# nantiferov/karpenter-sigs

Measured on AMD Instinct MI355X. Metric: pods/sec in Scheduler.Solve @50k pods x 400 types, higher is better.
Workload: dtype int64; 1 GPU; C2: 50000 resource-only pods x 400 fake.InstanceTypes, 1 NodeClaimTemplate, no limits, empty topology (BenchmarkScheduling shape); pods=50000, instance_types=400, parallelism=replicas1, new_nodeclaims=122

## Files before the change

### include/karpenter_amd.h

```cpp
#ifndef KARPENTER_AMD_H_
#define KARPENTER_AMD_H_

#include <stddef.h>
#include <stdint.h>

#ifdef __cplusplus
extern "C" {
#endif

#define KS_OK 0
#define KS_ERR_PARSE -1
#define KS_ERR_UNSUPPORTED -2
#define KS_ERR_CAPACITY -3
#define KS_ERR_HIP -4
#define KS_ERR_INTERNAL -5
#define KS_ERR_ARG -6

typedef struct ks_problem ks_problem;
typedef struct ks_results ks_results;

typedef struct ks_solve_opts {
  int device;
  int simulation_mode;
  int replicas;
  int timing_only;
  int lds_budget;
  int reserved[3];
} ks_solve_opts;

int ks_problem_create(const char* snapshot_json, size_t len, ks_problem** out);
void ks_problem_free(ks_problem* p);

int ks_problem_save(const ks_problem* p, void** buf, size_t* len);
int ks_problem_create_binary(const void* buf, size_t len, ks_problem** out);
int ks_snapshot_check(const char* snapshot_json, size_t len, size_t* bytes);
int ks_problem_encode_binary(const char* snapshot_json, size_t len, void** buf, size_t* blen);
int ks_problem_check_binary(const void* buf, size_t len);

int ks_problem_inspect(const char* snapshot_json, size_t len, char** dims_json);

int ks_problem_feasibility_rows(ks_problem* p, int which, char** meta_json, uint32_t** words, size_t* n_words);

int ks_problem_queue_inputs(const char* snapshot_json, size_t len, char** out_json);
int ks_problem_queue_readback(ks_problem* p, int32_t** order, int32_t** run_len, size_t* n, int* device_sorted);
int ks_claim_sort_probe(int device, int mode, int pos, int n, int R, int32_t* keys, int32_t* order,
                        const int32_t* claim_tpl, const int64_t* claim_head, int32_t* ptpl, int64_t* phead, int* how);
int ks_rec_headers_run(const int32_t* records, const int32_t* pass_ns, int n_passes, int TW, const int32_t* tpl_beg,
                       int ntpl, int32_t* headers, uint64_t* status, char** verdicts_json, char** meta_json);

int ks_solve(ks_problem* p, const ks_solve_opts* opts, ks_results** out);
void ks_results_free(ks_results* r);

int ks_results_json(const ks_results* r, char** json_out);

int ks_results_num_new_nodeclaims(const ks_results* r);
int ks_results_nodeclaim(const ks_results* r, int i, int* template_index, const int32_t** pods, int* n_pods,
                         const int32_t** instance_types, int* n_instance_types);
int ks_results_num_existing_nodes(const ks_results* r);
int ks_results_existing_node(const ks_results* r, int i, int* state_node_index, const int32_t** pods, int* n_pods);
int ks_results_num_pod_errors(const ks_results* r);
int ks_results_pod_error(const ks_results* r, int i, int* pod_index, const char** message);

typedef struct ks_requirement {
  const char* key;
  const char* op;
  int n_values;
  const char* const* values;
  int has_gt, has_lt;
  int64_t gt, lt;
} ks_requirement;
int ks_results_nodeclaim_requests(const ks_results* r, int i, int* n, const char* const** names,
                                  const char* const** quantities);
int ks_results_nodeclaim_requirements(const ks_results* r, int i, int* n, const ks_requirement** reqs);

double ks_results_kernel_ms(const ks_results* r);
double ks_results_solve_kernel_ms(const ks_results* r);
double ks_results_feasibility_ms(const ks_results* r);
double ks_results_feasibility_bytes(const ks_results* r);
double ks_results_node_feasibility_ms(const ks_results* r);
double ks_results_node_feasibility_bytes(const ks_results* r);
double ks_results_algorithmic_bytes(const ks_results* r);

typedef struct ks_cons ks_cons;
int ks_cons_create(const char* snapshot_json, size_t len, ks_cons** out);
int ks_cons_save(const ks_cons* c, void** buf, size_t* len);
int ks_cons_create_binary(const void* buf, size_t len, ks_cons** out);
int ks_cons_inspect(const char* snapshot_json, size_t len, char** out_json);
int ks_cons_update(ks_cons* c, const char* update_json, size_t len);
int ks_cons_inspect_update(const char* snapshot_json, size_t len, const char* update_json, size_t ulen,
                           char** out_json);
void ks_cons_free(ks_cons* c);
int ks_cons_num_candidates(const ks_cons* c);
int ks_cons_num_sims(const ks_cons* c);
int ks_cons_record_bytes(const ks_cons* c);
int ks_cons_records_per_rank(const ks_cons* c, int world);
int ks_cons_run(ks_cons* c, int rank, int world, const ks_solve_opts* opts, void* records, int records_on_device,
                double* kernel_ms);
#define KS_CONS_ALL_SIMS 1
#define KS_CONS_CANDIDATES 2
#define KS_CONS_NO_SIMS 4
int ks_cons_requirement_words(const ks_cons* c);
int ks_cons_needed_sims(ks_cons* c, const void* records, int world, int flags, int32_t* out, int cap);
int ks_cons_claim_requirements(ks_cons* c, int sim, uint32_t* out);
int ks_cons_decide(ks_cons* c, const void* records, int world, int flags, const uint32_t* rs_table,
                   char** json_out);
typedef struct ks_cons_clock {
  double multi_timeout_s;
  double single_timeout_s;
  double sim_seconds;
} ks_cons_clock;
int ks_cons_decide_clock(ks_cons* c, const void* records, int world, int flags, const uint32_t* rs_table,
                         const ks_cons_clock* clock, char** json_out);
int ks_cons_validate(ks_cons* c, const char* command_json, size_t len, const ks_solve_opts* opts, char** json_out);
#define KS_DISRUPT_EXPIRATION 1
#define KS_DISRUPT_DRIFT 2
int ks_cons_disrupt(ks_cons* c, int method, const ks_solve_opts* opts, int flags, char** json_out);
int ks_cons_inspect_disrupt(const char* snapshot_json, size_t len, const char* update_json, size_t ulen, int method,
                            char** out_json);
int ks_cons_encode_binary(const char* snapshot_json, size_t len, void** buf, size_t* buf_len);
int ks_cons_inspect_disrupt_binary(const void* buf, size_t len, int method, char** out_json, void** resaved,
                                   size_t* resaved_len);
int ks_cons_sim_counters(ks_cons* c, int sim, int64_t* out24);
int ks_cons_sim_counters_n(ks_cons* c, int sim, int64_t* out, int n);
int ks_cons_queue_readback(ks_cons* c, char** meta_json, int32_t** words, size_t* n_words);
int ks_cons_last_reruns(const ks_cons* c);
int ks_cons_last_routes(const ks_cons* c, char** json_out);
double ks_cons_records_alg_bytes(const ks_cons* c, const void* records, int world);

int ks_cluster_state(const char* cluster_json, size_t len, char** state_nodes_json);

void ks_free(void* p);
const char* ks_last_error(void);
int ks_device_count(void);
const char* ks_build_info(void);

#ifdef __cplusplus
}
#endif
#endif
```

### karpenter-sigs_amd/csrc/ks_capi.cpp

```cpp
#include <hip/hip_runtime_api.h>

#include <algorithm>
#include <chrono>
#include <cstring>
#include <memory>
#include <mutex>
#include <string>
#include <vector>

#include "../../include/karpenter_amd.h"
#include "ks_archive.h"
#include "ks_host.h"
#include "ks_runtime.h"
#include "ks_sort_probe.h"

using namespace ks;

static thread_local std::string g_err;
namespace ks {
void set_last_error(const std::string& m) { g_err = m; }

static thread_local std::vector<Route>* g_routes = nullptr;
void route_note(const Route& r) {
  if (g_routes) g_routes->push_back(r);
// ... 950 lines not shown
  return KS_OK;
  API_CATCH
}

extern "C++" {
namespace {
constexpr char kProblemMagic[8] = {'K', 'S', 'P', 'R', 'O', 'B', '0', '5'};
}

void snapshot_header(ArOut& a, const char magic[8]) {
  a.raw(magic, 8);
  uint32_t v[4] = {1u, (uint32_t)sizeof(KsDims), (uint32_t)sizeof(KeyMeta), (uint32_t)sizeof(Host)};
  a.raw(v, sizeof(v));
}
void snapshot_check_header(ArIn& a, const char magic[8]) {
  char m[8];
  uint32_t v[4];
  a.raw(m, 8);
  a.raw(v, sizeof(v));
  if (memcmp(m, magic, 6) == 0 && memcmp(m, magic, 8) != 0)
    throw KsError(KS_ERR_PARSE, "binary snapshot format version " + std::string(m + 6, 2) + ", this build reads version " +
                                    std::string(magic + 6, 2));
  if (memcmp(m, magic, 8) != 0) throw KsError(KS_ERR_PARSE, "not a binary snapshot of this kind");
  if (v[0] != 1u || v[1] != sizeof(KsDims) || v[2] != sizeof(KeyMeta) || v[3] != sizeof(Host))
    throw KsError(KS_ERR_PARSE, "binary snapshot from another build of the library");
}
char* snapshot_bytes(const std::string& s) {
  char* b = (char*)malloc(std::max<size_t>(s.size(), 1));
  if (!b) throw KsError(KS_ERR_CAPACITY, "out of host memory");
  memcpy(b, s.data(), s.size());
  return b;
}
}

int ks_problem_save(const ks_problem* p, void** buf, size_t* len) {
  API_TRY
  if (!p || !buf || !len) throw KsError(KS_ERR_ARG, "null argument");
  ArOut a;
  snapshot_header(a, kProblemMagic);
  host_save(a, const_cast<Host&>(p->host));
  *buf = snapshot_bytes(a.buf);
  *len = a.buf.size();
  return KS_OK;
  API_CATCH
}

int ks_problem_create_binary(const void* buf, size_t len, ks_problem** out) {
  API_TRY
  if (!buf || !out) throw KsError(KS_ERR_ARG, "null argument");
  std::unique_ptr<ks_problem> pb(new ks_problem());
  try {
    ArIn a{(const char*)buf, (const char*)buf + len};
    snapshot_check_header(a, kProblemMagic);
    host_load(a, pb->host);
    if (a.p != a.end) throw KsError(KS_ERR_PARSE, "binary snapshot has trailing bytes");
  } catch (const ArchiveError& e) {
    throw KsError(KS_ERR_PARSE, e.what());
  }
  problem_device_init(pb.get());
  *out = pb.release();
  return KS_OK;
  API_CATCH
}

int ks_snapshot_check(const char* json, size_t len, size_t* bytes) {
  API_TRY
  if (!json) throw KsError(KS_ERR_ARG, "null argument");
  PhaseTimer pt("ks_snapshot_check");
  ksjson::Value root = ksjson::Parser(json, len ? len : strlen(json)).parse();
  Host h;
  h.build(root);
  pt.mark("parse + encode");
  ArOut a;
  host_save(a, h);
  pt.mark("save");
  Host g;
  try {
    ArIn in{a.buf.data(), a.buf.data() + a.buf.size()};
    host_load(in, g);
    pt.mark("load");
    if (in.p != in.end) throw KsError(KS_ERR_INTERNAL, "snapshot reload left bytes");
  } catch (const ArchiveError& e) {
    throw KsError(KS_ERR_INTERNAL, e.what());
  }
  ArOut b;
  host_save(b, g);
  if (bytes) *bytes = a.buf.size();
  if (a.buf != b.buf) throw KsError(KS_ERR_INTERNAL, "snapshot save -> load -> save is not the identity");
  return KS_OK;
  API_CATCH
}

int ks_problem_encode_binary(const char* json, size_t len, void** buf, size_t* blen) {
  API_TRY
  if (!json || !buf || !blen) throw KsError(KS_ERR_ARG, "null argument");
  ksjson::Value root = ksjson::Parser(json, len ? len : strlen(json)).parse();
  Host h;
  h.build(root);
  ArOut a;
  snapshot_header(a, kProblemMagic);
  host_save(a, h);
  *buf = snapshot_bytes(a.buf);
  *blen = a.buf.size();
  return KS_OK;
  API_CATCH
}

int ks_problem_check_binary(const void* buf, size_t len) {
  API_TRY
  if (!buf) throw KsError(KS_ERR_ARG, "null argument");
  Host h;
  try {
    ArIn a{(const char*)buf, (const char*)buf + len};
    snapshot_check_header(a, kProblemMagic);
    host_load(a, h);
    if (a.p != a.end) throw KsError(KS_ERR_PARSE, "binary snapshot has trailing bytes");
  } catch (const ArchiveError& e) {
    throw KsError(KS_ERR_PARSE, e.what());
  }
  return KS_OK;
  API_CATCH
}

int ks_problem_inspect(const char* json, size_t len, char** out) {
  API_TRY
  if (!json || !out) throw KsError(KS_ERR_ARG, "null argument");
  ksjson::Value root = ksjson::Parser(json, len ? len : strlen(json)).parse();
  Host h;
  h.build(root);
  const KsDims& d = h.dims;
  std::string o = "{";
  auto kv = [&](const char* k, long long v) { o += std::string(o.size() > 1 ? "," : "") + "\"" + k + "\":" + std::to_string(v); };
  kv("R", d.R); kv("keys", d.NK); kv("W", d.W); kv("NB", d.NB); kv("RSW", d.RSW); kv("T", d.T); kv("templates", d.NTPL);
  kv("pools", d.NPOOL); kv("nodes", d.N); kv("pods", d.P); kv("states", d.S); kv("uids", d.NU); kv("TW", d.TW);
  kv("Kcap", d.Kcap); kv("taints", (long long)h.taints.size()); kv("G", d.G); kv("G1", d.G1);
  kv("hostQueue", h.hostQueue.empty() ? 0 : 1); kv("hostPorts", (long long)h.hostPortUniverse.size());
  long long nlate = 0;
  for (uint64_t x : h.tab.tg_late) nlate += __builtin_popcountll(x);
  kv("lateGroups", nlate); kv("groupWords", d.GMW); kv("unlabelledNodes", d.tgUnlab);
  kv("lean", d.lean); kv("negReq", d.negReq);
  long long nfail = 0, nshared = 0, nverr = 0;
  for (char x : h.injectFailed) nfail += x ? 1 : 0;
  for (int32_t f : h.tab.pod_flags) {
    nshared += (f & PF_VSHARED) ? 1 : 0;
    nverr += (f & PF_VOLERR) ? 1 : 0;
  }
  kv("volAny", d.volAny); kv("volDrivers", d.VD); kv("volPvcs", d.NVU); kv("volLogCap", d.vLogCap);
  kv("volSharedPods", nshared); kv("volErrorPods", nverr); kv("injectFailed", nfail);
  kv("volStaticMounts", (long long)(h.tab.pod_vsbeg.empty() ? 0 : h.tab.pod_vsbeg.back()));
  std::vector<int32_t> frontBeg, frontPos;
  pareto_fronts(d, h.tab.tpl_it_beg, h.tab.tpl_its, h.tab.it_alloc, frontBeg, frontPos);
  o += ",\"runFuse\":" + std::to_string(run_fuse_build()) + ",\"sortLeaf\":" + std::to_string(sort_leaf_build()) +
       ",\"closedShift\":" + std::to_string(closed_shift_build()) + ",\"tplMasks\":" + std::to_string(tpl_masks_build()) +
       ",\"logRuns\":" + std::to_string(log_runs_build()) + ",\"paretoFronts\":[";
  for (int t = 0; t < d.NTPL; t++) {
    o += t ? ",[" : "[";
    for (int i = frontBeg[(size_t)t]; i < frontBeg[(size_t)t + 1]; i++)
      o += (i > frontBeg[(size_t)t] ? "," : "") + std::to_string(frontPos[(size_t)i]);
    o += "]";
  }
  o += "]";
  o += ",\"plans\":{";
  const size_t budgets[] = {160 * 1024 - 256, 6000, 9000, 14000, 24000, 40000};
  long long fnr = 0;
  for (int32_t f : h.tab.st_flags) fnr += (f & SF_HAS_KEYS) ? 1 : 0;
  KsDims pd = d;
  pd.fnOn = node_rows_on(d, (size_t)fnr);
  auto plan_json = [&](size_t budget, int wide) {
    Plan pl = make_plan(pd, budget, false, wide, (int)frontPos.size());
    return "{\"KO\":" + std::to_string(pl.KO) +
           ",\"KL\":" + std::to_string(pl.KL) + ",\"talloc\":" + std::to_string(pl.talloc) +
           ",\"tsort\":" + std::to_string(pl.tsort) + ",\"tmask\":" + std::to_string(pl.tmask) +
           ",\"tmaskBytes\":" + std::to_string(pl.tmask ? tpl_mask_bytes(d.NTPL, d.TW) : 0) + ",\"lds\":" + std::to_string(pl.lds) + "}";
  };
  for (size_t i = 0; i < sizeof(budgets) / sizeof(budgets[0]); i++)
    o += (i ? ",\"" : "\"") + std::to_string(budgets[i]) + "\":" + plan_json(budgets[i], 0);
  o += "},\"widePlans\":{";
  for (size_t i = 0; i < sizeof(budgets) / sizeof(budgets[0]); i++)
    o += (i ? ",\"" : "\"") + std::to_string(budgets[i]) + "\":[" + plan_json(budgets[i], 1) + "," + plan_json(budgets[i], 2) + "]";
  o += "}";
  o += ",\"keyNames\":[";
  for (size_t i = 0; i < h.keyNames.size(); i++) { if (i) o += ","; ksjson::quote(o, h.keyNames[i]); }
  o += "],\"resources\":[";
  for (size_t i = 0; i < h.resNames.size(); i++) { if (i) o += ","; ksjson::quote(o, h.resNames[i]); }
  o += "],\"FNR\":" + std::to_string(fnr) + ",\"keyValues\":[";
  for (size_t i = 0; i < h.keys.size(); i++) o += (i ? "," : "") + std::to_string(h.keys[i].nv);
  o += "],\"coveredKeys\":[";
  bool firstKey = true;
  for (uint64_t m = d.itKeys & ~d.fkMulti; m; m &= m - 1) {
    if (!firstKey) o += ",";
    firstKey = false;
    ksjson::quote(o, h.keyNames[(size_t)__builtin_ctzll(m)]);
  }
  o += "]}";
  *out = strdup(o.c_str());
  return KS_OK;
  API_CATCH
}

int ks_problem_feasibility_rows(ks_problem* pb, int which, char** meta_json, uint32_t** words, size_t* n_words) {
  API_TRY
  if (!pb || !meta_json || !words || !n_words) throw KsError(KS_ERR_ARG, "null argument");
  if (which != 0 && which != 1) throw KsError(KS_ERR_ARG, "which must be 0 (instance-type rows) or 1 (node rows)");
  const Host& h = pb->host;
  const auto& t = h.tab;
  const KsDims& d = pb->dev.d;
  if (!(which == 0 ? d.fmOn : d.fnOn))
    throw KsError(KS_ERR_UNSUPPORTED, which == 0 ? "the instance-type rows are off for this problem"
                                                 : "the node rows are off for this problem");
  DeviceGuard guard(pb->device, nullptr);
  const size_t NWN = ((size_t)d.N + 31) / 32;
  const size_t n = which == 0 ? (size_t)d.S * d.NTPL * d.TW : (size_t)d.FNR * NWN;
  uint32_t* dst = which == 0 ? pb->dev.st_fm : pb->dev.st_fn;
  HIPCHK(hipMemsetAsync(dst, 0xA5, n * 4, pb->stream));
  if (which == 0)
    launch_feasibility(pb->dev, pb->stream);
  else
    launch_feasibility_nodes(pb->dev, pb->stream);
  HIPCHK(hipGetLastError());
  std::vector<uint32_t> host;
  dl(host, dst, n, pb->stream);
  HIPCHK(hipStreamSynchronize(pb->stream));
  std::string o = "{";
  auto kv = [&](const char* k, long long v) { o += std::string(o.size() > 1 ? "," : "") + "\"" + k + "\":" + std::to_string(v); };
  kv("S", d.S); kv("NTPL", d.NTPL); kv("TW", d.TW); kv("N", d.N); kv("FNR", d.FNR);
  auto ints = [&](const char* k, size_t cnt, auto&& at) {
    o += std::string(",\"") + k + "\":[";
    for (size_t i = 0; i < cnt; i++) o += (i ? "," : "") + std::to_string(at(i));
    o += "]";
  };
  ints("podState0", (size_t)d.P, [&](size_t i) { return (long long)t.pod_state0[i]; });
  ints("podNState", (size_t)d.P, [&](size_t i) { return (long long)t.pod_nstate[i]; });
  {
    int row = 0;
    ints("stateNodeRow", (size_t)d.S, [&](size_t s) { return (long long)((t.st_flags[s] & SF_HAS_KEYS) ? row++ : -1); });
  }
  ints("stateTolTpl", (size_t)d.S, [&](size_t s) { return (unsigned long long)t.st_toltpl[s]; });
  o += ",\"templates\":[";
  for (int tt = 0; tt < d.NTPL; tt++) {
    const int tb = t.tpl_it_beg[(size_t)tt], cnt = t.tpl_it_beg[(size_t)tt + 1] - tb;
    o += tt ? ",{\"instanceTypes\":[" : "{\"instanceTypes\":[";
    for (int p = 0; p < cnt; p++) {
      if (p) o += ",";
      ksjson::quote(o, h.its[(size_t)t.tpl_its[(size_t)(tb + p)]].name);
    }
    o += "],\"irregular\":[";
    const uint32_t* irr = &t.fk_words[(size_t)t.fk_tpl[(size_t)tt * 3 + 1]];
    for (int w = 0; w < d.TW; w++) o += (w ? "," : "") + std::to_string(irr[w]);
    o += "]}";
  }
  o += "],\"nodes\":[";
  for (int i = 0; i < d.N; i++) {
    if (i) o += ",";
    ksjson::quote(o, h.nodes[(size_t)i].name);
  }
  o += "],\"coveredKeys\":[";
  bool first = true;
  for (uint64_t m = d.itKeys & ~d.fkMulti; m; m &= m - 1) {
    if (!first) o += ",";
    first = false;
    ksjson::quote(o, h.keyNames[(size_t)__builtin_ctzll(m)]);
  }
  o += "]}";
  uint32_t* buf = (uint32_t*)malloc(std::max<size_t>(n, 1) * 4);
  if (!buf) throw KsError(KS_ERR_INTERNAL, "out of memory");
  memcpy(buf, host.data(), n * 4);
  *meta_json = strdup(o.c_str());
  *words = buf;
  *n_words = n;
  return KS_OK;
  API_CATCH
}

int ks_problem_queue_inputs(const char* json, size_t len, char** out) {
  API_TRY
  if (!json || !out) throw KsError(KS_ERR_ARG, "null argument");
  ksjson::Value root = ksjson::Parser(json, len ? len : strlen(json)).parse();
  Host h;
  h.build(root);
  *out = strdup((queue_inputs_json(h) + "}").c_str());
  return KS_OK;
  API_CATCH
}

int ks_problem_queue_readback(ks_problem* pb, int32_t** order, int32_t** run_len, size_t* n, int* device_sorted) {
  API_TRY
  if (!pb || !order || !run_len || !n || !device_sorted) throw KsError(KS_ERR_ARG, "null argument");
  const KsDims& d = pb->dev.d;
  DeviceGuard guard(pb->device, nullptr);
  const size_t P = (size_t)d.P, np = std::max<size_t>(P, 1), nw = (np + 63) / 64;
  struct Bufs {
    int32_t* qorder = nullptr;
    int32_t* rl = nullptr;
    uint64_t* words = nullptr;
    ~Bufs() {
      for (void* p : {(void*)qorder, (void*)rl, (void*)words})
        if (p) (void)hipFree(p);
    }
  } b;
  HIPCHK(hipMalloc((void**)&b.qorder, 4 * np));
  HIPCHK(hipMalloc((void**)&b.rl, 4 * np));
  HIPCHK(hipMalloc((void**)&b.words, 8 * nw));
  HIPCHK(hipMemsetAsync(b.qorder, 0xA5, 4 * np, pb->stream));
  HIPCHK(hipMemsetAsync(b.rl, 0xA5, 4 * np, pb->stream));
  HIPCHK(hipMemsetAsync(b.words, 0xA5, 8 * nw, pb->stream));
  HIPCHK(hipMemsetAsync(pb->skeys, 0xA5, 2 * np * sizeof(uint64_t), pb->stream));
  HIPCHK(hipMemsetAsync(pb->svals, 0xA5, 2 * np * sizeof(int32_t), pb->stream));
  const int32_t* fixed = pb->hqorder;
  if (!fixed) HIPCHK(queue_sort(pb->dev, pb->skeys, pb->svals, pb->stemp, pb->stempBytes, b.qorder, pb->stream));
  const bool lean = d.lean != 0;
  if (lean)
    HIPCHK(sim_run_lengths(fixed ? fixed : b.qorder, nullptr, pb->dev.pod_req, pb->dev.pod_s0, pb->dev.pod_flags, d.R,
                           d.P, b.words, b.rl, pb->stream, true));
  std::vector<int32_t> ho, hr;
  dl(ho, fixed ? fixed : b.qorder, P, pb->stream);
  if (lean) dl(hr, b.rl, P, pb->stream);
  HIPCHK(hipStreamSynchronize(pb->stream));
  int32_t* o = (int32_t*)malloc(4 * np);
  int32_t* r = lean ? (int32_t*)malloc(4 * np) : nullptr;
  if (!o || (lean && !r)) {
    free(o);
    free(r);
    throw KsError(KS_ERR_INTERNAL, "out of memory");
  }
  memcpy(o, ho.data(), 4 * P);
  if (lean) memcpy(r, hr.data(), 4 * P);
  *order = o;
  *run_len = r;
  *n = P;
  *device_sorted = fixed ? 0 : 1;
  return KS_OK;
  API_CATCH
}

int ks_claim_sort_probe(int device, int mode, int pos, int n, int R, int32_t* keys, int32_t* order,
                        const int32_t* claim_tpl, const int64_t* claim_head, int32_t* ptpl, int64_t* phead, int* how) {
  API_TRY
  if (const char* bad = sort_probe_check(mode, pos, n, R, keys, order, claim_tpl, claim_head, ptpl, phead))
    throw KsError(KS_ERR_ARG, bad);
  if (device < 0) {
    sort_probe_host(n, R, keys, order, claim_tpl, claim_head, ptpl, phead);
    if (how) *how = 1;
    return KS_OK;
  }
  DeviceGuard guard(device, nullptr);
  const size_t np = std::max<size_t>((size_t)n, 1);
  struct Bufs {
    int32_t *keys = nullptr, *order = nullptr, *ctpl = nullptr, *ptpl = nullptr, *how = nullptr;
    int64_t *chead = nullptr, *phead = nullptr;
    hipStream_t stream = nullptr;
    ~Bufs() {
      for (void* p : {(void*)keys, (void*)order, (void*)ctpl, (void*)ptpl, (void*)how, (void*)chead, (void*)phead})
        if (p) (void)hipFree(p);
      if (stream) (void)hipStreamDestroy(stream);
    }
  } b;
  HIPCHK(hipStreamCreateWithFlags(&b.stream, hipStreamNonBlocking));
  HIPCHK(hipMalloc((void**)&b.keys, 4 * np));
  HIPCHK(hipMalloc((void**)&b.order, 4 * np));
  HIPCHK(hipMalloc((void**)&b.ctpl, 4 * np));
  HIPCHK(hipMalloc((void**)&b.ptpl, 4 * np));
  HIPCHK(hipMalloc((void**)&b.how, 4 * kWave));
  HIPCHK(hipMalloc((void**)&b.chead, 8 * np * R));
  HIPCHK(hipMalloc((void**)&b.phead, 8 * np * R));
  HIPCHK(hipMemsetAsync(b.ptpl, 0xA5, 4 * np, b.stream));
  HIPCHK(hipMemsetAsync(b.phead, 0xA5, 8 * np * R, b.stream));
  HIPCHK(hipMemsetAsync(b.how, 0xA5, 4 * kWave, b.stream));
  if (n > 0) {
    HIPCHK(hipMemcpyAsync(b.keys, keys, 4 * (size_t)n, hipMemcpyHostToDevice, b.stream));
    HIPCHK(hipMemcpyAsync(b.order, order, 4 * (size_t)n, hipMemcpyHostToDevice, b.stream));
    HIPCHK(hipMemcpyAsync(b.ctpl, claim_tpl, 4 * (size_t)n, hipMemcpyHostToDevice, b.stream));
    HIPCHK(hipMemcpyAsync(b.chead, claim_head, 8 * (size_t)n * R, hipMemcpyHostToDevice, b.stream));
  }
  HIPCHK(claim_sort_probe(b.keys, b.order, n, mode, pos, R, b.ctpl, b.chead, b.ptpl, b.phead, b.how, b.stream));
  int32_t h = -1;
  if (n > 0) {
    HIPCHK(hipMemcpyAsync(keys, b.keys, 4 * (size_t)n, hipMemcpyDeviceToHost, b.stream));
    HIPCHK(hipMemcpyAsync(order, b.order, 4 * (size_t)n, hipMemcpyDeviceToHost, b.stream));
    HIPCHK(hipMemcpyAsync(ptpl, b.ptpl, 4 * (size_t)n, hipMemcpyDeviceToHost, b.stream));
    HIPCHK(hipMemcpyAsync(phead, b.phead, 8 * (size_t)n * R, hipMemcpyDeviceToHost, b.stream));
  }
  HIPCHK(hipMemcpyAsync(&h, b.how, 4, hipMemcpyDeviceToHost, b.stream));
  HIPCHK(hipStreamSynchronize(b.stream));
  if (how) *how = h;
  return KS_OK;
  API_CATCH
}

void ks_problem_free(ks_problem* p) {
  if (p && --p->refs == 0) delete p;
}
void ks_results_free(ks_results* r) { delete r; }

int ks_solve(ks_problem* pb, const ks_solve_opts* opts, ks_results** out) {
  API_TRY
  if (!pb || !out) throw KsError(KS_ERR_ARG, "null argument");
  int reps = opts && opts->replicas > 1 ? opts->replicas : 1;
  DeviceGuard guard(pb->device, opts);
  const KsDims& d = pb->host.dims;
  size_t budget = 160 * 1024 - 256;
  if (reps > 256) budget = std::max<size_t>(24 * 1024, budget * 256 / reps);
  if (opts && opts->lds_budget > 0) budget = std::min<size_t>(budget, (size_t)opts->lds_budget);
  Plan pl = make_plan(d, budget, false, pb->wideKO, pb->dev.frontTotal);
  if (pl.lds > 160 * 1024 || pl.KO < 1)
    throw KsError(KS_ERR_CAPACITY, "solve state does not fit the LDS budget");
  pb->lastKO = pl.KO;
  WorkLayout wl = work_layout(d);
  size_t need = wl.total * reps;
  if (need > pb->wbytes || reps != pb->wreps) {
    if (pb->wbuf) HIPCHK(hipFree(pb->wbuf));
    if (pb->works_dev) HIPCHK(hipFree(pb->works_dev));
    pb->wbuf = nullptr;
    pb->works_dev = nullptr;
    HIPCHK(hipMalloc(&pb->wbuf, need));
    HIPCHK(hipMalloc(&pb->works_dev, sizeof(KsWork) * reps));
    std::vector<KsWork> ws;
    for (int r = 0; r < reps; r++) ws.push_back(work_ptrs((char*)pb->wbuf + wl.total * r, wl));
    for (auto& x : ws) x.run_len = ws[0].run_len;
    HIPCHK(hipMemcpy(pb->works_dev, ws.data(), sizeof(KsWork) * reps, hipMemcpyHostToDevice));
    pb->wbytes = need;
    pb->wreps = reps;
  }
  KsWork w0 = work_ptrs((char*)pb->wbuf, wl);
  hipEvent_t e0, em, ep, e1, ef[4];
  HIPCHK(hipEventCreate(&e0));
  HIPCHK(hipEventCreate(&em));
  HIPCHK(hipEventCreate(&ep));
  HIPCHK(hipEventCreate(&e1));
  for (auto& e : ef) HIPCHK(hipEventCreate(&e));
  float ms = 0, setup = 0, post = 0, fms = 0, fnms = 0;
  int feasLaunches = 0, attempts = 0;
  int wide = pb->wideKO;
  std::vector<Route> routes;
  RouteScope routeScope(&routes);
  for (int attempt = 0; attempt < 4; attempt++) {
    attempts++;
    HIPCHK(hipEventRecord(e0, pb->stream));
    HIPCHK(launch_solve(pb->dev, pb->works_dev, reps, pl, w0.qorder, pb->skeys, pb->svals, pb->stemp,
                        pb->stempBytes, pb->stream, em, pb->hqorder, ef, (int32_t*)w0.run_len,
                        (uint64_t*)((char*)pb->wbuf + wl.run_words), ep));
    HIPCHK(hipEventRecord(e1, pb->stream));
    HIPCHK(hipEventSynchronize(e1));
    float a = 0, b = 0, f = 0;
    HIPCHK(hipEventElapsedTime(&a, e0, e1));
    HIPCHK(hipEventElapsedTime(&b, e0, em));
    float c = 0;
    HIPCHK(hipEventElapsedTime(&c, ep, e1));
    post += c;
    if (pb->dev.d.fmOn) {
      HIPCHK(hipEventElapsedTime(&f, ef[0], ef[1]));
      feasLaunches++;
    }
    if (pb->dev.d.fnOn) {
      float fn = 0;
      HIPCHK(hipEventElapsedTime(&fn, ef[2], ef[3]));
      fnms += fn;
    }
    ms += a;
    setup += b;
    fms += f;
    int64_t err = 0;
    HIPCHK(hipMemcpy(&err, w0.counters + CT_ERROR, 8, hipMemcpyDeviceToHost));
    if (err == KE_LEAN_EXIT && pb->dev.d.lean) {
      pb->dev.d.lean = 0;
      continue;
    }
    if (err != KE_CLAIM_CAP) break;
    int next = wide + 1;
    Plan np{};
    for (; next <= 2; next++) {
      np = make_plan(d, budget, false, next, pb->dev.frontTotal);
      if (np.lds <= 160 * 1024 && np.KO > pl.KO) break;
    }
    if (next > 2) break;
    pl = np;
    wide = pb->wideKO = next;
    pb->lastKO = pl.KO;
  }
  (void)hipEventDestroy(e0);
  (void)hipEventDestroy(em);
  (void)hipEventDestroy(ep);
  (void)hipEventDestroy(e1);
  for (auto& e : ef) (void)hipEventDestroy(e);
  ks_results* r;
  if (opts && opts->timing_only) {
    r = new ks_results();
    dl(r->counters, w0.counters, CT_NCOUNTERS, pb->stream);
    HIPCHK(hipStreamSynchronize(pb->stream));
    if (r->counters[CT_ERROR] != KE_OK) {
      const int64_t err = r->counters[CT_ERROR];
      delete r;
      if (err == KE_CLAIM_CAP) throw claim_cap_error(pb);
      throw KsError(KS_ERR_INTERNAL, "solve kernel reported error " + std::to_string(err));
    }
    r->algbytes = (double)r->counters[CT_ALGBYTES];
  } else {
    r = collect(pb, w0);
  }
  r->routes = routes;
  r->plan = pl;
  r->planWide = wide;
  r->kernel_ms = ms;
  r->solve_ms = ms - setup - post;
  r->feas_ms = fms;
  r->feas_bytes = pb->dev.d.fmOn ? pb->fmBytes * feasLaunches : 0;
  r->feasn_ms = fnms;
  r->feasn_bytes = pb->dev.d.fnOn ? pb->fnBytes * attempts : 0;
  *out = r;
  return KS_OK;
  API_CATCH
}

int ks_results_json(const ks_results* r, char** json_out) {
  API_TRY
  std::string o = "{\"newNodeClaims\":[";
  std::lock_guard<std::mutex> lk(r->render);
  for (size_t i = 0; i < r->claims.size(); i++) {
    finish_json(r->pb->host, r->claims[i]);
    o += (i ? "," : "") + r->claims[i].json;
  }
  o += "],\"existingNodes\":[";
  for (size_t i = 0; i < r->nodes.size(); i++) {
    o += i ? ",{\"name\":" : "{\"name\":";
    ksjson::quote(o, r->nodes[i].name);
    o += ",\"pods\":[";
    for (size_t k = 0; k < r->nodes[i].pods.size(); k++) o += (k ? "," : "") + std::to_string(r->nodes[i].pods[k]);
    o += "]}";
  }
  o += "],\"podErrors\":{";
  for (size_t i = 0; i < r->errors.size(); i++) {
    if (i) o += ",";
    ksjson::quote(o, std::to_string(r->errors[i].first));
    o += ":";
    ksjson::quote(o, r->errors[i].second);
  }
  o += "},\"stats\":{";
  static const char* names[] = {"nclaims", "ncommits", "hostnameCounter", "error", "pops", "algBytes",
                                "sorts", "sortsWithDescent", "claimFull", "claimQuickFail", "windows",
                                "cycPop", "cycNodes", "cycSort", "cycQuick", "cycFull", "cycCommit", "cycTemplates",
                                "cycTotal", "cycNodeCommit", "cycFullRs", "cycFullThr", "cycFullMasks", "cycFullApply",
                                "runs", "runPods", "sortsExact", "fineTopoPop", "fineState", "fineRefill",
                                "fineWindowTests", "fineWindowBlocks", "fineRecord", "fineNodeCommit", "fineWindowTopo",
                                "runCross", "runCrossStops", "runCrossLost", "sortsClosed", "tplMemoHits",
                                "cycSortFast", "cycSortExact", "cycSortClosed", "sortsLe12", "sortsLt50",
                                "cycRunCap", "cycCross", "cycBulk", "cycLog", "cycTplDerive", "cycTplStore",
                                "cycTplMax", "runCapFront", "runCapFull", "runCrossClosed", "runMoves",
                                "cycSortExactLe12", "cycSortExactLt50", "cycSortExactGe50", "closedShiftDiff",
                                "tplMaskFills", "tplMaskHits", "runRecs",
                                "cycTplCand", "cycTplFeas", "cycTplFilter", "cycTplThr", "cycLogLoad", "cycLogStore"};
  static_assert(sizeof(names) / sizeof(names[0]) == CT_NCOUNTERS, "one name per counter");
  for (int i = 0; i < CT_NCOUNTERS; i++) o += std::string(i ? "," : "") + "\"" + names[i] + "\":" + std::to_string(r->counters[i]);
  if (!r->routes.empty()) {
    std::string last = routes_json({r->routes.back()});
    o += ",\"route\":" + last.substr(1, last.size() - 3) + ",\"launches\":" + routes_json(r->routes) + "}";
  }
  o += ",\"plan\":{\"wide\":" + std::to_string(r->planWide) + ",\"KO\":" + std::to_string(r->plan.KO) +
       ",\"KL\":" + std::to_string(r->plan.KL) + ",\"talloc\":" + std::to_string(r->plan.talloc) +
       ",\"lds\":" + std::to_string(r->plan.lds) + "}";
  o += "}}";
  *json_out = strdup(o.c_str());
  return KS_OK;
  API_CATCH
}

int ks_results_num_new_nodeclaims(const ks_results* r) { return (int)r->claims.size(); }
int ks_results_nodeclaim(const ks_results* r, int i, int* tpl, const int32_t** pods, int* np, const int32_t** its, int* nit) {
  if (i < 0 || i >= (int)r->claims.size()) return KS_ERR_ARG;
  const auto& c = r->claims[i];
  if (tpl) *tpl = c.tpl;
  if (pods) *pods = c.pods.data();
  if (np) *np = (int)c.pods.size();
  if (its) *its = c.its.data();
  if (nit) *nit = (int)c.its.size();
  return KS_OK;
}
int ks_results_nodeclaim_requests(const ks_results* r, int i, int* n, const char* const** names,
                                  const char* const** quantities) {
  if (!r || i < 0 || i >= (int)r->claims.size()) return KS_ERR_ARG;
  const auto& c = r->claims[(size_t)i];
  if (n) *n = (int)c.reqNameP.size();
  if (names) *names = c.reqNameP.data();
  if (quantities) *quantities = c.reqQtyP.data();
  return KS_OK;
}
int ks_results_nodeclaim_requirements(const ks_results* r, int i, int* n, const ks_requirement** reqs) {
  if (!r || i < 0 || i >= (int)r->claims.size()) return KS_ERR_ARG;
  const auto& c = r->claims[(size_t)i];
  {
    std::lock_guard<std::mutex> lk(r->render);
    finish_reqs(r->pb->host, c);
  }
  if (n) *n = (int)c.reqC.size();
  if (reqs) *reqs = c.reqC.data();
  return KS_OK;
}
int ks_results_num_existing_nodes(const ks_results* r) { return (int)r->nodes.size(); }
int ks_results_existing_node(const ks_results* r, int i, int* idx, const int32_t** pods, int* np) {
  if (i < 0 || i >= (int)r->nodes.size()) return KS_ERR_ARG;
  if (idx) *idx = r->nodes[i].index;
  if (pods) *pods = r->nodes[i].pods.data();
  if (np) *np = (int)r->nodes[i].pods.size();
  return KS_OK;
}
int ks_results_num_pod_errors(const ks_results* r) { return (int)r->errors.size(); }
int ks_results_pod_error(const ks_results* r, int i, int* pod, const char** msg) {
  if (i < 0 || i >= (int)r->errors.size()) return KS_ERR_ARG;
  if (pod) *pod = r->errors[i].first;
  if (msg) *msg = r->errors[i].second.c_str();
  return KS_OK;
}
double ks_results_kernel_ms(const ks_results* r) { return r->kernel_ms; }
double ks_results_solve_kernel_ms(const ks_results* r) { return r->solve_ms; }
double ks_results_feasibility_ms(const ks_results* r) { return r->feas_ms; }
double ks_results_feasibility_bytes(const ks_results* r) { return r->feas_bytes; }
double ks_results_node_feasibility_ms(const ks_results* r) { return r->feasn_ms; }
double ks_results_node_feasibility_bytes(const ks_results* r) { return r->feasn_bytes; }
double ks_results_algorithmic_bytes(const ks_results* r) { return r->algbytes; }

}
```

### karpenter-sigs_amd/csrc/ks_problem.h

```cpp
#pragma once
#include <stdint.h>

#include "ks_reqset.h"

#if defined(__HIP_DEVICE_COMPILE__)
#define KS_G __attribute__((address_space(1)))
#define KS_L __attribute__((address_space(3)))
#define KS_C __attribute__((address_space(4)))
#else
#define KS_G
#define KS_L
#define KS_C
#endif

namespace ks {

constexpr int kMaxR = 16;
constexpr int kProbeMaxN = 1024;
constexpr int kMaxTpl = 64;
constexpr int kWave = 64;

enum PodStatus : int32_t { ST_PENDING = 0, ST_SCHEDULED = 1, ST_FAILED = 2 };
enum FailCode : uint32_t {
  FC_NONE = 0,
// ... 112 lines not shown
  const double KS_G* off_price;
  const uint64_t KS_G* pod_hpc;
  const uint64_t KS_G* pod_hpu;
  const uint64_t KS_G* pod_hpo;
  const uint64_t KS_G* n_hp0;
  const int32_t KS_G* tg_meta;
  const int32_t KS_G* tg_cnt0;
  const uint32_t KS_G* tg_frs;
  const uint64_t KS_G* st_gown;
  const uint64_t KS_G* pod_gsel;
  const uint64_t KS_G* pod_ginv;
  const uint64_t KS_G* tg_late;
  const uint32_t KS_G* st_rss;
  const int32_t KS_G* n_tdom;
  const uint32_t KS_G* fk_words;
  const int32_t KS_G* fk_key_off;
  const int32_t KS_G* fk_tpl;
  uint32_t KS_G* st_fm;
  const int32_t KS_G* st_fnrow;
  const int32_t KS_G* fn_state;
  uint32_t KS_G* st_fn;
  const int32_t KS_G* pod_vdbeg;
  const int32_t KS_G* pod_vd;
  const int32_t KS_G* pod_vsbeg;
  const int32_t KS_G* pod_vs;
  const int32_t KS_G* pod_vubeg;
  const int32_t KS_G* pod_vu;
  const int32_t KS_G* vol_udrv;
  const int32_t KS_G* n_vc0;
  const int32_t KS_G* n_vlim;
  const int32_t KS_G* tpl_front_beg;
  const int32_t KS_G* tpl_front;
  int32_t frontTotal;
};

enum NodeFlag : int32_t { NF_UNUSABLE = 1 };
enum TopoGroupType : int32_t { TG_SPREAD = 0, TG_AFFINITY = 1, TG_ANTI = 2 };
enum TgMeta : int32_t {
  TGM_TYPE = 0, TGM_KEY, TGM_SKEW, TGM_MIND, TGM_CNT, TGM_NV, TGM_FBEG, TGM_FEND, TGM_HOST,
  TGM_KSLOT,
  TGM_WORDS = 12
};
enum PodFlag : int32_t {
  PF_PROVISIONABLE = 1,
  PF_VSHARED = 2,
  PF_VOLERR = 4,
};
enum ConsFlag : int32_t { CF_PRICE_ERR = 1, CF_ALL_SPOT = 2, CF_MULTI = 4 };
enum ConsAction : int32_t { CA_NOOP = 0, CA_DELETE = 1, CA_REPLACE = 2, CA_ERROR = 3 };

enum RecField {
  RF_FLAGS = 0,
  RF_NCLAIMS,
  RF_HOSTINCR,
  RF_TPL,
  RF_HOST,
  RF_ACTION,
  RF_NOPT,
  RF_NPRICE,
  RF_NSAME,
  RF_ERROR,
  RF_ALGB_LO,
  RF_ALGB_HI,
  RF_CLAIM,
  RF_HDR = 16,
};
enum RecBit { RB_ALL_SCHEDULED = 1, RB_NARROWED = 2, RB_HAS_SPOT = 4, RB_HAS_OD = 8, RB_RELAXED = 16 };
KS_HD int rec_words(int TW) { return RF_HDR + 3 * TW; }

struct KsWork {
  int32_t KS_G* c_tpl;
  int32_t KS_G* c_cnt;
  int32_t KS_G* c_thr;
  int32_t KS_G* c_host;
  int64_t KS_G* c_req;
  int64_t KS_G* c_max;
  uint32_t KS_G* c_rs;
  uint32_t KS_G* c_rem;
  int32_t KS_G* order;
  int64_t KS_G* n_req;
  uint32_t KS_G* n_rs;
  int32_t KS_G* queue;
  int32_t KS_G* qorder;
  int32_t KS_G* pod_state;
  uint64_t KS_G* last_len;
  int32_t KS_G* log_pod;
  int32_t KS_G* log_tgt;
  int32_t KS_G* pod_status;
  int32_t KS_G* pod_fstate;
  uint32_t KS_G* fail_code;
  int32_t KS_G* fail_host;
  int64_t KS_G* pool_rem;
  int64_t KS_G* counters;
  uint64_t KS_G* n_hp;
  uint64_t KS_G* c_hp;
  int32_t KS_G* n_vc;
  int32_t KS_G* tg_cnt;
  int32_t KS_G* tg_cpos;
  int32_t KS_G* tg_ccnt;
  uint32_t KS_G* fail_rs;
  uint64_t KS_G* log_hg;
  int32_t KS_G* tg_act;
  const int32_t KS_G* pod_map;
  const int32_t KS_G* run_len;
  int32_t P;
  int32_t nrm;
  const int32_t KS_G* rm;
  const int64_t KS_G* pool0;
  const double KS_G* st_price;
  int32_t KS_G* rec;
  int32_t KS_G* n_slot;
  double price;
  int32_t cflags;
  int32_t ccs;
  const int32_t KS_G* tdel;
  int32_t ntdel;
  const uint64_t KS_G* tdead;
  const uint64_t KS_G* tact;
  const int32_t KS_G* sstart;
  const int32_t KS_G* tmd;
  int32_t ntmd;
  int32_t KS_G* n_vslot;
  int32_t KS_G* vlog;
  int32_t KS_G* vspec;
  int32_t KS_G* run_log;
};

enum Counter {
  CT_NCLAIMS = 0, CT_NLOG, CT_HOSTCTR, CT_ERROR, CT_POPS, CT_ALGBYTES, CT_SORTS, CT_SORT_SLOW,
  CT_CLAIM_FULL, CT_CLAIM_QUICK_FAIL, CT_WINDOWS,
  CT_CYC_POP, CT_CYC_NODES, CT_CYC_SORT, CT_CYC_QUICK, CT_CYC_FULL, CT_CYC_COMMIT, CT_CYC_TPL, CT_CYC_TOTAL,
  CT_CYC_NCOMMIT,
  CT_CYC_SUB,
  CT_ABI = 24,
  CT_RUNS = 24,
  CT_RUN_PODS,
  CT_SORT_EXACT,
  CT_FINE,
  CT_RUN_CROSS = CT_FINE + 8,
  CT_RUN_CROSS_STOPS,
  CT_RUN_CROSS_LOST,
  CT_SORT_CLOSED,
  CT_TPL_MEMO_HITS,
  CT_STEP,
  CT_RUN_CAP_FRONT = CT_STEP + 12,
  CT_RUN_CAP_FULL,
  CT_RUN_CROSS_CLOSED,
  CT_RUN_MOVES,
  CT_CYC_EXACT_BY_N,
  CT_CLOSED_SHIFT_DIFF = CT_CYC_EXACT_BY_N + 3,
  CT_TPL_MASK_FILLS,
  CT_TPL_MASK_HITS,
  CT_RUN_RECS,
  CT_CYC_SPLIT,
  CT_CYC_SPLIT_END = CT_CYC_SPLIT + 6,
  CT_NCOUNTERS = CT_CYC_SPLIT_END
};
enum SplitSub { YS_TPL_CAND = 0, YS_TPL_FEAS, YS_TPL_FILTER, YS_TPL_THR, YS_LOG_LOAD, YS_LOG_STORE };

enum StepSub {
  SS_SORT_FAST = 0,
  SS_SORT_EXACT,
  SS_SORT_CLOSED,
  SS_SORTS_LE12,
  SS_SORTS_LT50,
  SS_RUN_CAP,
  SS_CROSS,
  SS_BULK,
  SS_LOG,
  SS_TPL_DERIVE,
  SS_TPL_STORE,
  SS_TPL_MAX,
};
enum KernelError { KE_OK = 0, KE_CLAIM_CAP = 1, KE_ITER_CAP = 2, KE_STACK = 3, KE_LEAN_EXIT = 4 };

}
```

### karpenter-sigs_amd/csrc/ks_queue.hip

```cpp
#include <hip/hip_runtime.h>

#include <hipcub/hipcub.hpp>

#include "ks_problem.h"

namespace ks {

__global__ void k_qkeys(const int64_t* sortkey, int comp, int64_t minv, const int32_t* perm, uint64_t* keys,
                        int32_t* vals, int n, int first) {
  const int i = blockIdx.x * blockDim.x + threadIdx.x;
  if (i >= n) return;
  const int p = first ? i : perm[i];
  keys[i] = (uint64_t)(sortkey[(int64_t)p * 4 + comp] - minv);
  vals[i] = p;
}

__global__ void k_iota(int32_t* v, int n) {
  const int i = blockIdx.x * blockDim.x + threadIdx.x;
  if (i < n) v[i] = i;
}

size_t queue_sort_temp_bytes(int n) {
  size_t bytes = 0;
  (void)hipcub::DeviceRadixSort::SortPairs(nullptr, bytes, (const uint64_t*)nullptr, (uint64_t*)nullptr,
                                     (const int32_t*)nullptr, (int32_t*)nullptr, n, 0, 64, (hipStream_t)0);
  return bytes;
}

hipError_t queue_sort(const KsDev& D, uint64_t* keys, int32_t* vals, void* temp, size_t tempBytes,
                      int32_t* out, hipStream_t st) {
  const KsDims& d = D.d;
  const int n = d.P;
  if (n == 0) return hipSuccess;
  const int blocks = (n + 255) / 256;
  const int32_t* cur = nullptr;
  int buf = 0;
  for (int comp = 3; comp >= 0; comp--) {
    const int bits = d.skBits[comp];
    if (bits == 0) continue;
    uint64_t* kin = keys + (size_t)buf * n;
    int32_t* vin = vals + (size_t)buf * n;
    uint64_t* kout = keys + (size_t)(buf ^ 1) * n;
    int32_t* vout = vals + (size_t)(buf ^ 1) * n;
    hipLaunchKernelGGL(k_qkeys, dim3(blocks), dim3(256), 0, st, D.pod_sortkey, comp, d.skMin[comp], cur, kin, vin, n,
                       cur == nullptr ? 1 : 0);
    size_t tb = tempBytes;
    hipError_t e = hipcub::DeviceRadixSort::SortPairs(temp, tb, kin, kout, vin, vout, n, 0, bits, st);
    if (e != hipSuccess) return e;
    cur = vout;
    buf ^= 1;
  }
  if (cur == nullptr) {
    hipLaunchKernelGGL(k_iota, dim3(blocks), dim3(256), 0, st, out, n);
  } else {
    hipError_t e = hipMemcpyAsync(out, cur, sizeof(int32_t) * n, hipMemcpyDeviceToDevice, st);
    if (e != hipSuccess) return e;
  }
  return hipGetLastError();
}

__global__ void k_sim_keys(const int32_t* rank, const int32_t* entries, const int32_t* entry_sim, int rbits,
                           uint64_t* keys, int32_t* vals, int n) {
  const int i = blockIdx.x * blockDim.x + threadIdx.x;
  if (i >= n) return;
  const int p = entries[i];
  keys[i] = ((uint64_t)entry_sim[i] << rbits) | (uint64_t)rank[p];
  vals[i] = p;
}

__global__ void k_rank(const int32_t* order, int32_t* rank, int n) {
  const int i = blockIdx.x * blockDim.x + threadIdx.x;
  if (i < n) rank[order[i]] = i;
}

hipError_t rank_from_order(const int32_t* order, int32_t* rank, int n, hipStream_t st) {
  if (n == 0) return hipSuccess;
  hipLaunchKernelGGL(k_rank, dim3((n + 255) / 256), dim3(256), 0, st, order, rank, n);
  return hipGetLastError();
}

hipError_t sim_queue_sort(const int32_t* rank, const int32_t* entries, const int32_t* entry_sim, int n, int rbits,
                          int sbits, uint64_t* keys, int32_t* vals, void* temp, size_t tempBytes, int32_t* out,
                          hipStream_t st) {
  if (n == 0) return hipSuccess;
  hipLaunchKernelGGL(k_sim_keys, dim3((n + 255) / 256), dim3(256), 0, st, rank, entries, entry_sim, rbits, keys, vals, n);
  size_t tb = tempBytes;
  return hipcub::DeviceRadixSort::SortPairs(temp, tb, keys, keys + n, vals, out, n, 0, rbits + sbits, st);
}

__global__ __launch_bounds__(256) void k_sim_run_breaks(const int32_t* podmap, const int32_t* entry_sim,
                                                        const int64_t* pod_req, const uint64_t* pod_s0,
                                                        const int32_t* pod_flags, int R, int n, uint64_t* words,
                                                        int strict) {
  const int i = blockIdx.x * blockDim.x + threadIdx.x;
  bool brk = true;
  if (i < n && i > 0 && (!entry_sim || entry_sim[i] == entry_sim[i - 1])) {
    const int p = podmap[i], q = podmap[i - 1];
    bool same = pod_s0[4 * (int64_t)p] == pod_s0[4 * (int64_t)q] && pod_s0[4 * (int64_t)p + 1] == pod_s0[4 * (int64_t)q + 1] &&
                ((pod_flags[p] ^ pod_flags[q]) & PF_PROVISIONABLE) == 0;
    if (strict)
      same = same && pod_s0[4 * (int64_t)p + 2] == pod_s0[4 * (int64_t)q + 2] &&
             pod_s0[4 * (int64_t)p + 3] == pod_s0[4 * (int64_t)q + 3];
    for (int r = 0; r < R; r++) same = same && pod_req[(int64_t)p * R + r] == pod_req[(int64_t)q * R + r];
    brk = !same;
  }
  const uint64_t b = __ballot(brk ? 1 : 0);
  if ((threadIdx.x & 63) == 0 && i < n) words[i >> 6] = b;
}

__global__ __launch_bounds__(256) void k_sim_run_len(const uint64_t* words, int n, int32_t* run_len) {
  const int i = blockIdx.x * blockDim.x + threadIdx.x;
  if (i >= n) return;
  const int nw = (n + 63) >> 6;
  int w = (i + 1) >> 6;
  uint64_t m = w < nw ? words[w] & (~0ull << ((i + 1) & 63)) : 0ull;
  while (m == 0 && ++w < nw) m = words[w];
  const int next = m ? (w << 6) + __builtin_ctzll(m) : n;
  run_len[i] = (next < n ? next : n) - i;
}

hipError_t sim_run_lengths(const int32_t* podmap, const int32_t* entry_sim, const int64_t* pod_req, const uint64_t* pod_s0,
                           const int32_t* pod_flags, int R, int n, uint64_t* words, int32_t* run_len, hipStream_t st,
                           bool strict) {
  if (n == 0) return hipSuccess;
  const int blocks = (n + 255) / 256;
  hipLaunchKernelGGL(k_sim_run_breaks, dim3(blocks), dim3(256), 0, st, podmap, entry_sim, pod_req, pod_s0, pod_flags, R,
                     n, words, strict ? 1 : 0);
  hipLaunchKernelGGL(k_sim_run_len, dim3(blocks), dim3(256), 0, st, words, n, run_len);
  return hipGetLastError();
}

}

namespace ks {

__global__ __launch_bounds__(256) void k_rec_headers(const int32_t* recs, int ns, int recWords, int TW,
                                                     const int32_t* tplBeg, int ntpl, int32_t* hdr,
                                                     unsigned long long* status, unsigned* counter,
                                                     unsigned long long* statusOut) {
  __shared__ int32_t tile[256 * (RF_HDR + 1)];
  __shared__ unsigned last;
  const int s0 = blockIdx.x * blockDim.x, s = s0 + threadIdx.x;
  if (s < ns) {
    const int32_t* r = recs + (size_t)s * recWords;
    int32_t h[RF_HDR];
    for (int i = 0; i < RF_HDR; i++) {
      h[i] = r[i];
      tile[threadIdx.x * (RF_HDR + 1) + i] = h[i];
    }
    int bad = 0;
    if (h[RF_ACTION] < CA_NOOP || h[RF_ACTION] > CA_ERROR) bad = 1;
    else if (h[RF_NCLAIMS] < 0 || h[RF_HOSTINCR] < h[RF_NCLAIMS]) bad = 2;
    else if (h[RF_ACTION] == CA_DELETE && h[RF_NCLAIMS] != 0) bad = 3;
    else if (h[RF_ACTION] == CA_REPLACE && h[RF_NCLAIMS] != 1) bad = 4;
    else if (h[RF_NCLAIMS] > 0) {
      if (h[RF_TPL] < 0 || h[RF_TPL] >= ntpl) {
        bad = 5;
      } else {
        const int nIT = tplBeg[h[RF_TPL] + 1] - tplBeg[h[RF_TPL]];
        const uint32_t* o = (const uint32_t*)r + RF_HDR;
        int nopt = 0, nprice = 0, nsame = 0;
        for (int w = 0; w < TW; w++) {
          const int lo = w * 32;
          const uint32_t valid = nIT >= lo + 32 ? ~0u : nIT > lo ? (1u << (nIT - lo)) - 1u : 0u;
          const uint32_t a = o[w], b = o[TW + w], c = o[2 * TW + w];
          if (a & ~valid) bad = 6;
          if ((b & ~a) || (c & ~b)) bad = bad ? bad : 7;
          nopt += __popc(a);
          nprice += __popc(b);
          nsame += __popc(c);
        }
        if (!bad && (nopt != h[RF_NOPT] || nopt == 0)) bad = 8;
        if (!bad && (nprice != h[RF_NPRICE] || nsame != h[RF_NSAME])) bad = 9;
      }
    }
    if (bad) atomicMin(status, ((unsigned long long)s << 32) | (unsigned)bad);
    if (h[RF_ERROR] != KE_OK) atomicMin(status + 1, ((unsigned long long)s << 32) | (unsigned)h[RF_ERROR]);
  }
  __syncthreads();
  const int nb = ns - s0 < (int)blockDim.x ? ns - s0 : (int)blockDim.x;
  for (int w = threadIdx.x; w < nb * RF_HDR; w += blockDim.x)
    hdr[(size_t)s0 * RF_HDR + w] = tile[(w / RF_HDR) * (RF_HDR + 1) + w % RF_HDR];
  __threadfence();
  __syncthreads();
  if (threadIdx.x == 0) last = atomicAdd(counter, 1u) == gridDim.x - 1 ? 1u : 0u;
  __syncthreads();
  if (last && threadIdx.x < 2) {
// ... 17 lines not shown
```

### karpenter-sigs_amd/csrc/ks_runtime.h

```cpp
#pragma once
#include <atomic>
#include <hip/hip_runtime_api.h>

#include <string>
#include <vector>

#include "../../include/karpenter_amd.h"
#include "ks_host.h"
#include "ks_tplmask.h"

namespace ks {
hipError_t launch_solve(const KsDev& D, const KsWork* works_dev, int nrep, const Plan& pl, int32_t* qorder,
                        uint64_t* skeys, int32_t* svals, void* stemp, size_t stempBytes, hipStream_t st,
                        hipEvent_t mid, const int32_t* fixed_order = nullptr, hipEvent_t* feas = nullptr,
                        int32_t* run_len = nullptr, uint64_t* run_words = nullptr, hipEvent_t post = nullptr);
hipError_t launch_sims(const KsDev& D, const KsWork* works_dev, int nsims, const Plan& pl, hipStream_t st);
hipError_t launch_sims_topo(const KsDev& D, const KsWork* w, int n, const Plan& pl, hipStream_t st);
void launch_feasibility(const KsDev& D, hipStream_t st);
void launch_feasibility_nodes(const KsDev& D, hipStream_t st);
bool sims_mw_supported(const KsDev& D, const Plan& pl);
hipError_t launch_sims_split(const KsDev& D, const KsWork* works_dev, int nsims, int nmw, const Plan& pl, hipStream_t st,
                             hipStream_t st2, hipEvent_t fork, hipEvent_t join);
int run_fuse_build();
int sort_leaf_build();
int closed_shift_build();
int tpl_masks_build();
int log_runs_build();
hipError_t claim_sort_probe(int32_t* keys, int32_t* order, int n, int mode, int pos, int R, const int32_t* ctpl,
                            const int64_t* chead, int32_t* ptpl, int64_t* phead, int32_t* how, hipStream_t st);
Plan make_plan(const KsDims& d, size_t budget, bool sim = false, int wideKO = 0, int frontTotal = 0);
size_t queue_sort_temp_bytes(int n);
hipError_t queue_sort(const KsDev& D, uint64_t* keys, int32_t* vals, void* temp, size_t tempBytes, int32_t* out,
                      hipStream_t st);
hipError_t rank_from_order(const int32_t* order, int32_t* rank, int n, hipStream_t st);
hipError_t rec_headers(const int32_t* recs, int ns, int recWords, int TW, const int32_t* tplBeg, int ntpl, int32_t* hdr,
                       unsigned long long* status, unsigned* counter, unsigned long long* statusOut, hipStream_t st);
hipError_t sim_run_lengths(const int32_t* podmap, const int32_t* entry_sim, const int64_t* pod_req, const uint64_t* pod_s0,
                           const int32_t* pod_flags, int R, int n, uint64_t* words, int32_t* run_len, hipStream_t st,
                           bool strict = false);
hipError_t sim_queue_sort(const int32_t* rank, const int32_t* entries, const int32_t* entry_sim, int n, int rbits,
                          int sbits, uint64_t* keys, int32_t* vals, void* temp, size_t tempBytes, int32_t* out,
                          hipStream_t st);

std::vector<uint64_t> pod_first_state_words(const Host& h);
std::string queue_inputs_json(const Host& h);

struct Arena {
  size_t total = 0;
  size_t add(size_t bytes) {
    size_t off = total;
    total += (bytes + 255) & ~(size_t)255;
    return off;
  }
};

void set_last_error(const std::string& m);

struct RouteScope {
  std::vector<Route>* prev;
  explicit RouteScope(std::vector<Route>* log);
  ~RouteScope();
  RouteScope(const RouteScope&) = delete;
  RouteScope& operator=(const RouteScope&) = delete;
};
std::string routes_json(const std::vector<Route>& log);
}

#define HIPCHK(x)                                                                                         \
  do {                                                                                                    \
    hipError_t e_ = (x);                                                                                  \
    if (e_ != hipSuccess) throw ks::KsError(KS_ERR_HIP, std::string(#x) + ": " + hipGetErrorString(e_)); \
  } while (0)

struct ks_problem {
  std::atomic<int> refs{1};
  ks::Host host;
  ks::KsDev dev{};
  void* dbuf = nullptr;
  void* fmbuf = nullptr;
  double fmBytes = 0;
  void* fnbuf = nullptr;
  double fnBytes = 0;
  void* wbuf = nullptr;
  size_t wbytes = 0;
  ks::KsWork* works_dev = nullptr;
  int wreps = 0;
  hipStream_t stream = nullptr;
  int device = -1;
  int lastKO = 0;
  int wideKO = 0;
  uint64_t* skeys = nullptr;
  int32_t* svals = nullptr;
  void* stemp = nullptr;
  size_t stempBytes = 0;
  int32_t* hqorder = nullptr;
  ~ks_problem() {
    int prev = -1;
    if (device >= 0 && hipGetDevice(&prev) == hipSuccess && prev != device) (void)hipSetDevice(device);
    if (skeys) (void)hipFree(skeys);
    if (svals) (void)hipFree(svals);
    if (stemp) (void)hipFree(stemp);
    if (hqorder) (void)hipFree(hqorder);
    if (dbuf) (void)hipFree(dbuf);
    if (fmbuf) (void)hipFree(fmbuf);
    if (fnbuf) (void)hipFree(fnbuf);
    if (wbuf) (void)hipFree(wbuf);
    if (works_dev) (void)hipFree(works_dev);
    if (stream) (void)hipStreamDestroy(stream);
    if (prev >= 0 && prev != device) (void)hipSetDevice(prev);
  }
};

namespace ks {
struct DeviceGuard {
  int prev = -1;
  DeviceGuard(int dev, const ks_solve_opts* opts) {
    if (opts && opts->device >= 0 && opts->device != dev)
      throw KsError(KS_ERR_ARG, "opts->device " + std::to_string(opts->device) + " is not the device the handle was created on (" +
                                    std::to_string(dev) + ")");
    HIPCHK(hipGetDevice(&prev));
    if (prev != dev) HIPCHK(hipSetDevice(dev));
    (void)hipGetLastError();
  }
  ~DeviceGuard() {
    if (prev >= 0) (void)hipSetDevice(prev);
  }
  DeviceGuard(const DeviceGuard&) = delete;
  DeviceGuard& operator=(const DeviceGuard&) = delete;
};
}

void ks_upload(ks_problem* pb);

namespace ks { struct ArOut; struct ArIn; }
void snapshot_header(ks::ArOut& a, const char magic[8]);
void snapshot_check_header(ks::ArIn& a, const char magic[8]);
char* snapshot_bytes(const std::string& s);

#define API_TRY try {
#define API_CATCH                                  \
  }                                                \
  catch (const ks::KsError& e) {                   \
    ks::set_last_error(e.what());                  \
    return e.code;                                 \
  }                                                \
  catch (const std::exception& e) {                \
    ks::set_last_error(e.what());                  \
    return KS_ERR_PARSE;                           \
  }
```

### karpenter-sigs_amd/csrc/ks_solve.hip

```cpp
#include <hip/hip_runtime.h>

#ifndef KS_FM_OFF
#define KS_FM_OFF 0
#endif
#ifndef KS_TU
#define KS_TU 0
#endif
#ifndef KS_RUN_MIN
#define KS_RUN_MIN 3
#endif
#ifndef KS_NODE_K
#define KS_NODE_K 2
#endif
#ifndef KS_SORT_LANE0
#define KS_SORT_LANE0 0
#endif
#ifndef KS_SORT_LEAF
#define KS_SORT_LEAF 1
#endif
#ifndef KS_CLAIM_RUNS
#define KS_CLAIM_RUNS 1
#endif
#ifndef KS_RUN_CROSS
#define KS_RUN_CROSS 1
#endif
#ifndef KS_RUN_FRONT
#define KS_RUN_FRONT 1
#endif
#ifndef KS_RUN_FUSE
#define KS_RUN_FUSE 0
#endif
#ifndef KS_CLOSED_SHIFT
#define KS_CLOSED_SHIFT 0
#endif
#ifndef KS_SORT_CLOSED
#define KS_SORT_CLOSED 1
#endif
#ifndef KS_SORT_OUTLINE
#define KS_SORT_OUTLINE 1
#endif
#ifndef KS_TPL_MEMO
#define KS_TPL_MEMO 1
#endif
#ifndef KS_LOG_AHEAD
#define KS_LOG_AHEAD 0
#endif
#ifndef KS_TPL_MASKS
#define KS_TPL_MASKS 0
#endif
#ifndef KS_LOG_RUNS
#define KS_LOG_RUNS 1
#endif

#include "ks_gosort.h"
#include "ks_problem.h"
#include "ks_reqset.h"
#include "ks_tplmask.h"

namespace ks {

using LI32 = int32_t KS_L*;
using LI64 = int64_t KS_L*;
using LU32 = uint32_t KS_L*;
using LU64 = uint64_t KS_L*;
using GI32 = int32_t KS_G*;
using GI64 = int64_t KS_G*;
using GU32 = uint32_t KS_G*;
using DevLayout = ReqLayoutT<const KeyMeta KS_L*, const uint32_t KS_G*, const int64_t KS_G*>;
enum GroupSet : int { GS_MASK = 0, GS_SEL, GS_INV, GS_ACT, GS_N };

__device__ __forceinline__ int lane() { return (int)threadIdx.x & (kWave - 1); }
__device__ __forceinline__ uint64_t wballot(bool p) { return __ballot(p ? 1 : 0); }
__device__ __forceinline__ int ctz64(uint64_t m) { return __builtin_ctzll(m); }
__device__ __forceinline__ int popc64(uint64_t m) { return __popcll(m); }
__device__ __forceinline__ int uni(int x) { return __builtin_amdgcn_readfirstlane(x); }
__device__ __forceinline__ bool ub(bool x) { return __builtin_amdgcn_readfirstlane((int)x) != 0; }
__device__ __forceinline__ int64_t uni64(int64_t x) {
  return (int64_t)(((uint64_t)(uint32_t)__builtin_amdgcn_readfirstlane((int)(x >> 32)) << 32) |
                   (uint32_t)__builtin_amdgcn_readfirstlane((int)x));
}
__device__ __forceinline__ int rdl(int x, int l) { return __builtin_amdgcn_readlane(x, l); }
__device__ __forceinline__ int64_t rdl64(int64_t x, int l) {
  return (int64_t)(((uint64_t)(uint32_t)__builtin_amdgcn_readlane((int)(x >> 32), l) << 32) |
                   (uint32_t)__builtin_amdgcn_readlane((int)x, l));
}
__device__ __forceinline__ void wsync() {
  __builtin_amdgcn_fence(__ATOMIC_SEQ_CST, "wavefront");
  __builtin_amdgcn_wave_barrier();
}
__device__ __forceinline__ void hbm_release() { __builtin_amdgcn_fence(__ATOMIC_RELEASE, "workgroup"); }
template <class T>
__device__ __forceinline__ T ld_sc1(const T KS_G* p) {
  return __hip_atomic_load((T*)p, __ATOMIC_RELAXED, __HIP_MEMORY_SCOPE_AGENT);
}
__device__ __forceinline__ uint32_t lds_and(LU32 p, uint32_t v) {
  return __hip_atomic_fetch_and(p, v, __ATOMIC_RELAXED, __HIP_MEMORY_SCOPE_WAVEFRONT);
}
__device__ __forceinline__ int wscan_add(int v) {
  v += __builtin_amdgcn_update_dpp(0, v, 0x111, 0xf, 0xf, false);
  v += __builtin_amdgcn_update_dpp(0, v, 0x112, 0xf, 0xf, false);
  v += __builtin_amdgcn_update_dpp(0, v, 0x114, 0xf, 0xf, false);
  v += __builtin_amdgcn_update_dpp(0, v, 0x118, 0xf, 0xf, false);
  const int r0 = __builtin_amdgcn_readlane(v, 15), r1 = r0 + __builtin_amdgcn_readlane(v, 31);
  const int r2 = r1 + __builtin_amdgcn_readlane(v, 47), l = lane();
  return v + (l >= 48 ? r2 : l >= 32 ? r1 : l >= 16 ? r0 : 0);
}
__device__ __forceinline__ int wscan_max(int v) {
  auto mx = [](int a, int b) { return a > b ? a : b; };
  v = mx(v, __builtin_amdgcn_update_dpp(-1, v, 0x111, 0xf, 0xf, false));
  v = mx(v, __builtin_amdgcn_update_dpp(-1, v, 0x112, 0xf, 0xf, false));
  v = mx(v, __builtin_amdgcn_update_dpp(-1, v, 0x114, 0xf, 0xf, false));
  v = mx(v, __builtin_amdgcn_update_dpp(-1, v, 0x118, 0xf, 0xf, false));
  const int r0 = __builtin_amdgcn_readlane(v, 15), r1 = mx(r0, __builtin_amdgcn_readlane(v, 31));
  const int r2 = mx(r1, __builtin_amdgcn_readlane(v, 47)), l = lane();
  return mx(v, l >= 48 ? r2 : l >= 32 ? r1 : l >= 16 ? r0 : -1);
}
template <int CTRL>
__device__ __forceinline__ int dpp32(int old, int v) { return __builtin_amdgcn_update_dpp(old, v, CTRL, 0xf, 0xf, false); }
template <int CTRL>
__device__ __forceinline__ int64_t dpp64(int64_t old, int64_t v) {
  const int lo = dpp32<CTRL>((int)old, (int)v), hi = dpp32<CTRL>((int)(old >> 32), (int)(v >> 32));
  return (int64_t)(((uint64_t)(uint32_t)hi << 32) | (uint32_t)lo);
}
template <int CTRL> __device__ __forceinline__ int dppT(int old, int v) { return dpp32<CTRL>(old, v); }
template <int CTRL> __device__ __forceinline__ uint32_t dppT(uint32_t old, uint32_t v) { return (uint32_t)dpp32<CTRL>((int)old, (int)v); }
template <int CTRL> __device__ __forceinline__ int64_t dppT(int64_t old, int64_t v) { return dpp64<CTRL>(old, v); }
template <int CTRL> __device__ __forceinline__ uint64_t dppT(uint64_t old, uint64_t v) { return (uint64_t)dpp64<CTRL>((int64_t)old, (int64_t)v); }
__device__ __forceinline__ int rdlT(int x, int l) { return rdl(x, l); }
__device__ __forceinline__ uint32_t rdlT(uint32_t x, int l) { return (uint32_t)rdl((int)x, l); }
__device__ __forceinline__ int64_t rdlT(int64_t x, int l) { return rdl64(x, l); }
__device__ __forceinline__ uint64_t rdlT(uint64_t x, int l) { return (uint64_t)rdl64((int64_t)x, l); }
template <class T, class F>
__device__ __forceinline__ T wred(T v, T fill, F op) {
  v = op(v, dppT<0x111>(fill, v));
  v = op(v, dppT<0x112>(fill, v));
  v = op(v, dppT<0x114>(fill, v));
  v = op(v, dppT<0x118>(fill, v));
  return op(op(rdlT(v, 15), rdlT(v, 31)), op(rdlT(v, 47), rdlT(v, 63)));
}
template <class T> __device__ __forceinline__ T wred_min(T v, T fill) { return wred(v, fill, [](T a, T b) { return b < a ? b : a; }); }
template <class T> __device__ __forceinline__ T wred_max(T v, T fill) { return wred(v, fill, [](T a, T b) { return b > a ? b : a; }); }
template <class T> __device__ __forceinline__ T wred_add(T v) { return wred(v, (T)0, [](T a, T b) { return a + b; }); }
__device__ __forceinline__ float run_rcp(int64_t req) { return req > 0 ? __builtin_amdgcn_rcpf((float)req) : 0.f; }
__device__ __forceinline__ int run_cap(int64_t free, int64_t req, float rq, int m) {
  if (req == 0) return free >= 0 ? m : 0;
  if (req == 1) return free <= 0 ? 0 : (free < (int64_t)m ? (int)free : m);
  const float q = fminf((float)free * rq, (float)(m + 2));
  int qi = q > 0.f ? (int)q : 0;
  qi -= (int64_t)qi * req > free ? 1 : 0;
  qi += (int64_t)(qi + 1) * req <= free ? 1 : 0;
  qi = qi < m ? qi : m;
  return free >= req ? qi : 0;
}

template <int U, class T>
__device__ __forceinline__ void lds_copy(T KS_L* dst, const T KS_G* src, int n) {
  int i = lane();
  for (; i + (U - 1) * kWave < n; i += U * kWave) {
    T v[U];
#pragma unroll
    for (int u = 0; u < U; u++) v[u] = src[i + u * kWave];
#pragma unroll
    for (int u = 0; u < U; u++) dst[i + u * kWave] = v[u];
  }
  for (; i < n; i += kWave) dst[i] = src[i];
}

#ifdef KS_PHASE_STATS
#define PH_BEGIN(v) uint64_t v = __builtin_amdgcn_s_memtime()
#define PH_END(v, slot) cyc[slot] += __builtin_amdgcn_s_memtime() - v
#define PHS_END(v, slot) scyc[slot] += __builtin_amdgcn_s_memtime() - v
#define SPHS_END(o, v, slot) o.scyc[slot] += __builtin_amdgcn_s_memtime() - v
#define FPH_END(v, slot) fcyc[slot] += __builtin_amdgcn_s_memtime() - v
#define XPH_END(v, slot) xcyc[slot] += __builtin_amdgcn_s_memtime() - v
#define SXPH_END(o, v, slot) o.xcyc[slot] += __builtin_amdgcn_s_memtime() - v
#define XPH_COUNT(slot) xcyc[slot] += 1
#define YPH_END(v, slot) ycyc[slot] += __builtin_amdgcn_s_memtime() - v
#define SYPH_END(o, v, slot) o.ycyc[slot] += __builtin_amdgcn_s_memtime() - v
#define PH_WAIT_LOADS() __builtin_amdgcn_s_waitcnt(0x0f70)
#else
#define PH_BEGIN(v)
#define PH_END(v, slot)
#define PHS_END(v, slot)
#define SPHS_END(o, v, slot)
#define FPH_END(v, slot)
#define XPH_END(v, slot)
#define SXPH_END(o, v, slot)
#define XPH_COUNT(slot)
#define YPH_END(v, slot)
#define SYPH_END(o, v, slot)
#define PH_WAIT_LOADS()
#endif

#if KS_TU == 0
__global__ void k_init(KsDev D, const KsWork* works, int nrep, const int32_t* qorder) {
  const KsDims d = D.d;
  const int64_t gtid = (int64_t)blockIdx.x * blockDim.x + threadIdx.x;
  const int64_t gsz = (int64_t)gridDim.x * blockDim.x;
  for (int r = 0; r < nrep; r++) {
    const KsWork W = works[r];
    for (int64_t i = gtid; i < (int64_t)d.N * d.R; i += gsz) W.n_req[i] = D.n_req0[i];
    for (int64_t i = gtid; i < (int64_t)d.N * d.RSW; i += gsz) W.n_rs[i] = D.n_rs0[i];
    for (int64_t i = gtid; i < d.N; i += gsz) W.n_hp[i] = D.n_hp0[i];
    if (d.volAny)
      for (int64_t i = gtid; i < (int64_t)d.N * d.VD; i += gsz) W.n_vc[i] = D.n_vc0[i];
    if (d.G) {
      for (int64_t i = gtid; i < d.tgCntWords; i += gsz) W.tg_cnt[i] = D.tg_cnt0[i];
      for (int64_t i = gtid; i < (int64_t)d.G * (d.Kcap + 1); i += gsz) W.tg_ccnt[i] = 0;
      for (int64_t i = gtid; i < d.G; i += gsz) W.tg_cpos[i] = 0;
// ... 536 lines not shown
    for (int u = 0; u < 4; u++) {
      const int q = pc + 1 + u * kWave + lane(), k = s_okey[q < n ? q : n - 1];
      kq[u] = q < n ? k : INT32_MAX;
    }
    pv = w_choose_pivot(0, n, hint);
    if (!cand || hint != 1 || !ub(K > nx)) return -1;
    int t = 0;
    bool end = false;
#pragma unroll
    for (int u = 0; u < 4; u++) {
      const uint64_t m = wballot(kq[u] < K);
      t += end ? 0 : popc64(m);
      end = end || m != ~0ull;
    }
    for (int base = pos + 1 + 4 * kWave; !end && base < n; base += 4 * kWave) {
      uint64_t m[4];
#pragma unroll
      for (int u = 0; u < 4; u++) {
        const int q = base + u * kWave + lane();
        m[u] = wballot(q < n && s_okey[q] < K);
      }
#pragma unroll
      for (int u = 0; u < 4; u++) {
        t += end ? 0 : popc64(m[u]);
        end = end || m[u] != ~0ull;
      }
    }
    const int to = pos + t;
    const int v0 = s_order[pos], tp0 = ptpl[pos];
    int64_t h0[R];
#pragma unroll
    for (int r = 0; r < R; r++) h0[r] = phead[(int64_t)pos * R + r];
    for (int lo = pos + 1; lo <= to; lo += 4 * kWave) {
      int k[4], v[4], tp[4];
      int64_t h[4][R];
      const int nu = (to - lo) / kWave + 1;
#pragma unroll
      for (int u = 0; u < 4; u++) {
        if (u < nu) {
          const int j = lo + u * kWave + lane(), jj = j <= to ? j : to;
          k[u] = s_okey[jj];
          v[u] = s_order[jj];
          tp[u] = ptpl[jj];
#pragma unroll
          for (int r = 0; r < R; r++) h[u][r] = phead[(int64_t)jj * R + r];
        }
      }
      wsync();
#pragma unroll
      for (int u = 0; u < 4; u++) {
        const int j = lo + u * kWave + lane();
        if (u < nu && j <= to) {
          s_okey[j - 1] = k[u];
          s_order[j - 1] = v[u];
          ptpl[j - 1] = tp[u];
#pragma unroll
          for (int r = 0; r < R; r++) phead[(int64_t)(j - 1) * R + r] = h[u][r];
        }
      }
      wsync();
    }
    s_okey[to] = K;
    s_order[to] = v0;
    ptpl[to] = tp0;
#pragma unroll
    for (int r = 0; r < R; r++) phead[(int64_t)to * R + r] = h0[r];
    wsync();
    return t;
  }
  template <bool LEAF>
  __device__ void w_pdqsort(int n, int resumePivot) {
    int fa = 0, fb = 0, fl = 0, ff = 0;
    int sp = 0;
    {
      const bool me = lane() == 0;
      fa = me ? 0 : fa;
      fb = me ? n : fb;
      fl = me ? GoSortT<LI32>::bitsLen((uint32_t)n) : fl;
      ff = me ? 3 : ff;
      sp = 1;
    }
    bool resume = resumePivot >= 0;
    int dummy_lo = 0, dummy_hi = 0;
    while (sp > 0) {
      sp--;
      int a = rdl(fa, sp), b = rdl(fb, sp), limit = rdl(fl, sp);
      const int flags = rdl(ff, sp);
      bool wasBalanced = flags & 1, wasPartitioned = (flags >> 1) & 1;
      for (;;) {
        const int length = b - a;
        int pivot;
        if (resume) {
          resume = false;
          pivot = resumePivot;
        } else {
          if (KS_SORT_LEAF && LEAF && length <= 12) {
            w_leaf(a, b);
            break;
          }
          if (length <= 12 || limit == 0) {
            if (lane() == 0) {
              GoSortT<LI32> g{s_okey, s_order};
              if (length <= 12) g.insertionSort(a, b);
              else g.heapSort(a, b);
            }
            wsync();
            break;
          }
          if (!wasBalanced) {
            if (lane() == 0) {
              GoSortT<LI32> g{s_okey, s_order};
              g.breakPatterns(a, b);
            }
            wsync();
            limit--;
          }
          int hint = 0;
          pivot = w_choose_pivot(a, b, hint);
          if (hint == 2) {
            w_reverse(a, b);
            pivot = (b - 1) - (pivot - a);
            hint = 1;
          }
          if (wasBalanced && wasPartitioned && hint == 1 && pis_wave(a, b, dummy_lo, dummy_hi)) break;
        }
        if (a > 0 && ub(!(s_okey[a - 1] < s_okey[pivot]))) {
          a = w_partition_equal(a, b, pivot);
          continue;
        }
        bool already = false;
        const int mid = w_partition(a, b, pivot, already);
        wasPartitioned = already;
        const int leftLen = mid - a, rightLen = b - mid, thr = length / 8;
        if (sp + 2 > kWave) return;
        int c0a, c0b, c1a, c1b;
        if (leftLen < rightLen) {
          wasBalanced = leftLen >= thr;
          c0a = mid + 1; c0b = b; c1a = a; c1b = mid;
        } else {
          wasBalanced = rightLen >= thr;
          c0a = a; c0b = mid; c1a = mid + 1; c1b = b;
        }
        const bool m0 = lane() == sp, m1 = lane() == sp + 1;
        fa = m0 ? c0a : (m1 ? c1a : fa);
        fb = m0 ? c0b : (m1 ? c1b : fb);
        fl = (m0 || m1) ? limit : fl;
        ff = m0 ? ((int)wasBalanced | ((int)wasPartitioned << 1)) : (m1 ? 3 : ff);
        sp += 2;
        break;
      }
    }
  }
};
template <bool LEAF>
static __device__ __forceinline__ uint32_t claim_sort_general(LI32 okey, LI32 order, int n, int pivot) {
  ClaimSort cs;
  cs.s_order = order;
  cs.s_okey = okey;
  int tlo = n, thi = -1;
  bool done = false;
  if (pivot >= 0) done = cs.pis_wave(0, n, tlo, thi);
  if (!done) {
#if KS_SORT_LANE0
    if (lane() == 0) {
      GoSortExactT<LI32> g{GoSortT<LI32>{okey, order}};
      g.run(n, pivot);
    }
#else
    cs.template w_pdqsort<LEAF>(n, pivot);
#endif
    tlo = 0;
    thi = n - 1;
  }
  return (uint32_t)tlo | (uint32_t)(thi + 1) << 15 | (uint32_t)done << 30;
}
static __device__ __noinline__ uint32_t claim_sort_general_out(LI32 okey, LI32 order, int n, int pivot) {
  return claim_sort_general<true>(okey, order, n, pivot);
}

template <int RT, bool TL, bool SIM, bool TOPO, bool LEAN>
struct Solver : ClaimSort {
  static constexpr int RM = RT > 0 ? RT : kMaxR;
  static_assert(!(LEAN && TOPO), "LEAN excludes topology");
  __device__ __forceinline__ bool hpA() const { return !LEAN && d.hpAny; }
  __device__ __forceinline__ bool volA() const { return !LEAN && d.volAny; }
  __device__ __forceinline__ bool negR() const { return !LEAN && d.negReq; }
  __device__ __forceinline__ bool dupU() const { return !LEAN && d.dupUids; }
  __device__ __forceinline__ bool keys(int sflags) const { return !LEAN && (sflags & SF_HAS_KEYS); }
  const KsDev& D;
  const KsDims& d;
  const KsWork KS_C& W;
  const Plan& pl;
  DevLayout L;
  ClaimView<true> lc;
  ClaimView<false> gc;
  LI32 s_ptpl;
  LI64 s_phead;
  LI64 s_talloc;
  LI64 s_tsa;
  LI32 s_tsp;
  LI32 s_tbeg;
  LI64 s_pool;
  LU32 s_rs;
  LU32 s_pin;
  LU32 s_rem;
  LU32 s_cand;
  LU32 s_fic;
  LU32 s_fof;
  LU32 s_firr;
  enum : int { MM_T = 0, MM_CNT, MM_FOK, MM_POD = 4 };
  static constexpr bool TPL_MEMO = KS_TPL_MEMO && LEAN && !SIM;
  LU32 s_memo;
  int64_t memoHits = 0;
  static constexpr bool TPL_MASKS = KS_TPL_MASKS && LEAN && !SIM;
  LU32 s_tmask;
  LU32 s_tmv;
  int64_t maskFills = 0, maskHits = 0;
  static constexpr bool RUN_FRONT = KS_RUN_FRONT && KS_CLAIM_RUNS && LEAN && !SIM;
  enum : int { TPL_FOK = 1 << 30 };
  static __device__ __forceinline__ int tplv(int x) { return RUN_FRONT ? x & ~(int)TPL_FOK : x; }
  LI32 s_fbeg;
  LI32 s_front;
  mutable int64_t capFront = 0, capFull = 0;
  LU32 s_rmv;
  LU32 s_tch;
  LU32 s_tchr;
  LU32 s_tvol;
  LI32 s_tgm;
  LI32 s_tmin;
  LU32 s_trs0;
  LU32 s_trs1;
  LI32 s_tdom;
  LI32 s_tdw;
  LI32 s_live;
  LI32 s_tcs;
  LU32 s_tcd;
  LU64 s_gw;
  uint64_t t_mask = 0;
  uint64_t t_sel = 0;
  uint64_t t_inv = 0;
  bool t_any = false;
  bool t_rec = false;
  int t_s = 0;
  uint64_t t_rss = 0;
  const uint32_t KS_G* fnp = nullptr;
  bool t_nonode = false;
  uint64_t t_active = ~0ull;
  int64_t algbytes = 0;
  bool rem_same = false;
  uint64_t cur_hpc = 0, cur_hpu = 0;
  uint64_t cur_hpo = 0;
  enum : int { VO_DB = 0, VO_DE, VO_SB, VO_SE, VO_NSP, VO_UB, VO_UE, VO_NLOG, VO_NSLOT, VO_WORDS };
  LI32 s_vol;
#ifdef KS_PHASE_STATS
  mutable uint64_t scyc[4] = {0, 0, 0, 0};
  mutable uint64_t xcyc[12] = {0, 0, 0, 0, 0, 0, 0, 0, 0, 0, 0, 0};
  uint64_t ecyc[3] = {0, 0, 0};
  mutable uint64_t ycyc[6] = {0, 0, 0, 0, 0, 0};
#endif

  __device__ Solver(const KsDev& D_, const KsWork KS_C& W_, const Plan& p_) : D(D_), d(D_.d), W(W_), pl(p_) {}
  __device__ __forceinline__ int R() const { return RT > 0 ? RT : d.R; }

  template <bool INL>
  __device__ __forceinline__ const ClaimView<INL>& cv() const {
    if constexpr (INL) return lc;
    else return gc;
  }

  template <class P>
  __device__ __forceinline__ bool fits(const int64_t* req, P alloc) const {
    bool ok = true;
#pragma unroll
    for (int r = 0; r < RM; r++) {
      if (RT == 0 && r >= d.R) break;
      const int64_t a = alloc[r];
      ok &= (a >= 0) & (req[r] <= a);
    }
    return ok;
  }
  __device__ __forceinline__ bool fits_pos(const int64_t* req, int gpos) const {
    if constexpr (TL) return fits(req, s_talloc + (int64_t)gpos * R());
    else return fits(req, D.it_alloc + (int64_t)D.tpl_its[gpos] * R());
  }
  __device__ __forceinline__ int64_t alloc_pos(int gpos, int r) const {
    if constexpr (TL) return s_talloc[(int64_t)gpos * R() + r];
    else return D.it_alloc[(int64_t)D.tpl_its[gpos] * R() + r];
  }
  __device__ __forceinline__ int64_t tsort_a(int64_t i) const {
    if constexpr (TL) return s_tsa[i];
    else return D.tsort_alloc[i];
  }
  __device__ __forceinline__ int tsort_p(int64_t i) const {
    if constexpr (TL) return s_tsp[i];
    else return D.tsort_pos[i];
  }

  int lg_p = 0, lg_t = 0;
  static constexpr bool LOG_RUNS = KS_LOG_RUNS && KS_CLAIM_RUNS && LEAN && !SIM;
  int lg_lo = 0;
  int runRecs = 0;
  __device__ __forceinline__ void log_commit(int p, int tgt, int& nlog) {
    if constexpr (SIM) {
      nlog++;
      return;
    }
    if (lane() == (nlog & (kWave - 1))) {
      lg_p = p;
      lg_t = tgt;
    }
    nlog++;
    if ((nlog & (kWave - 1)) == 0) {
      if (!LOG_RUNS || lane() >= lg_lo) {
        W.log_pod[nlog - kWave + lane()] = lg_p;
        W.log_tgt[nlog - kWave + lane()] = lg_t;
      }
      if constexpr (LOG_RUNS) lg_lo = 0;
    }
  }
  __device__ __forceinline__ void log_batch(int n, int pod_t, int tgt_t, int& nlog) {
    if constexpr (SIM) {
      nlog += n;
      return;
    }
    const int b0 = nlog & (kWave - 1);
    const int src = (lane() - b0) & (kWave - 1);
    const int pv = __shfl(pod_t, src), tv = __shfl(tgt_t, src);
    const bool mine = src < n;
    if (mine && lane() >= b0) {
      lg_p = pv;
// ... 1183 lines not shown
              if (nclaims >= pl.KO) return -1;
              const int c = nclaims++;
              XPH_END(ttd, SS_TPL_DERIVE);
              PH_BEGIN(tts0);
              if (SIM && TOPO)
                for (int g = lane(); g < d.G; g += kWave) W.tg_ccnt[(int64_t)g * W.ccs + nclaims] = 0;
              const bool inl = c < pl.KL;
              copy_words(W.c_rs + (int64_t)c * d.RSW, s_rs, d.RSW);
              if (inl) copy_words(lc.rem + (int64_t)c * d.TW, s_rem, d.TW);
              else copy_words(gc.rem + (int64_t)c * d.TW, s_rem, d.TW);
              XPH_END(tts0, SS_TPL_STORE);
              PH_BEGIN(ttd1);
              int thr[RM];
              for (int r = 0; r < R(); r++) {
                if (hit) {
                  thr[r] = uni((int)s_memo[MM_POD + 4 * R() + r]);
                  continue;
                }
                const int64_t b = (int64_t)tb * R() + (int64_t)r * nIT;
                int k = 0;
                for (int q = 0; q < nIT; q += kWave)
                  k += __popcll(wballot(q + lane() < nIT && tsort_a(b + q + lane()) < req[r]));
                thr[r] = k;
              }
              const int cnt = hit ? uni((int)s_memo[MM_CNT]) : popc_words(s_rem, d.TW);
              bool fok = false;
              if constexpr (RUN_FRONT) {
                if (hit) {
                  fok = uni((int)s_memo[MM_FOK]) != 0;
                } else {
                  const int fb = s_fbeg[t], nf = s_fbeg[t + 1] - fb;
                  const int q = lane() < nf ? s_front[fb + lane()] : 0;
                  const bool miss = lane() < nf && fits_pos(req, tb + q) && !((s_rem[q >> 5] >> (q & 31)) & 1u);
                  fok = nf > 0 && wballot(miss) == 0;
                }
              }
              XPH_END(ttd1, SS_TPL_DERIVE);
              YPH_END(ttd1, YS_TPL_THR);
              PH_BEGIN(tts1);
              for (int r = 0; r < R(); r++) {
                if (inl) {
                  lc.req[(int64_t)c * R() + r] = req[r];
                  lc.thr[(int64_t)c * R() + r] = thr[r];
                } else {
                  gc.req[(int64_t)c * R() + r] = req[r];
                  gc.thr[(int64_t)c * R() + r] = thr[r];
                }
              }
              if (inl) {
                lc.tpl[c] = RUN_FRONT && fok ? t | (int)TPL_FOK : t;
                lc.cnt[c] = cnt;
              } else {
                gc.cnt[c] = cnt;
              }
              W.c_tpl[c] = t;
              W.c_hp[c] = cur_hpu;
              W.c_host[c] = hostid;
              s_order[c] = c;
              s_okey[c] = 1;
              s_ptpl[c] = t;
              srt = c == 0 || uni(s_okey[c - 1]) <= 1;
              log_commit(p, c, nlog);
              hbm_release();
              wsync();
              XPH_END(tts1, SS_TPL_STORE);
              if (TOPO && t_rec) topo_record(s_rs, c, -1, d.allowWK, nlog - 1);
              PH_BEGIN(ttm);
              if (hit) {
                const LI64 mx = (LI64)(s_memo + MM_POD + 2 * R());
                for (int r = 0; r < R(); r++) {
                  const int64_t m = uni64(mx[r]);
                  if (inl) lc.max[(int64_t)c * R() + r] = m;
                  else gc.max[(int64_t)c * R() + r] = m;
                  s_phead[(int64_t)c * R() + r] = m - req[r];
                }
                if (!inl) hbm_release();
                wsync();
                memoHits++;
              } else {
                if (mk) maskHits++;
                if (inl) recompute_max<true>(c, s_rem, t, c);
                else recompute_max<false>(c, s_rem, t, c);
                if constexpr (TPL_MEMO) {
                  if (pool < 0 && !d.fmOn) {
                    const LI64 mp = (LI64)(s_memo + MM_POD);
                    for (int r = 0; r < R(); r++) {
                      mp[r] = pod[r];
                      mp[R() + r] = inl ? uni64(lc.max[(int64_t)c * R() + r]) : uni64(ld_sc1(gc.max + (int64_t)c * R() + r));
                      s_memo[MM_POD + 4 * R() + r] = (uint32_t)thr[r];
                    }
                    copy_words(s_memo + MM_POD + 5 * R(), s_rem, d.TW);
                    s_memo[MM_T] = (uint32_t)t;
                    s_memo[MM_CNT] = (uint32_t)cnt;
                    if constexpr (RUN_FRONT) s_memo[MM_FOK] = fok ? 1u : 0u;
                    wsync();
                  }
                }
              }
              XPH_END(ttm, SS_TPL_MAX);
              if (pool >= 0) {
                const uint32_t mask = D.pool_mask[pool];
                for (int r = 0; r < R(); r++) {
                  if (!((mask >> r) & 1u)) continue;
                  int64_t m = INT64_MIN;
                  for (int pos = lane(); pos < nIT; pos += kWave)
                    if ((s_rem[pos >> 5] >> (pos & 31)) & 1u) {
                      const int64_t v = D.it_cap[(int64_t)D.tpl_its[tb + pos] * R() + r];
                      m = v > m ? v : m;
                    }
                  m = wred_max(m, (int64_t)INT64_MIN);
                  s_pool[(int64_t)pool * R() + r] -= m;
                }
                wsync();
              }
              return 1;
            }
          }
        }
      }
      W.fail_code[(int64_t)p * d.NTPL + t] = code;
      W.fail_host[(int64_t)p * d.NTPL + t] = hostid;
    }
    return 0;
  }

  __device__ __forceinline__ int sim_template_calls(int& hostCtr) const {
    for (int t = 0; t < d.NTPL; t++) {
      const int pool = D.tpl_pool[t];
      bool call = pool < 0;
      if (!call) {
        const int tb = s_tbeg[t], nIT = s_tbeg[t + 1] - tb;
        const uint32_t mask = D.pool_mask[pool];
        uint64_t anyCand = 0;
        for (int base = 0; base < nIT && !anyCand; base += kWave) {
          const int pos = base + lane();
          bool ok = pos < nIT;
          if (ok) {
            const int64_t KS_G* cap = D.it_cap + (int64_t)D.tpl_its[tb + pos] * R();
            for (int r = 0; r < R(); r++)
              ok = ok && !(((mask >> r) & 1u) && cap[r] > s_pool[(int64_t)pool * R() + r]);
          }
          anyCand = wballot(ok);
        }
        call = anyCand != 0;
      }
      if (call) hostCtr = uni(hostCtr + 1);
    }
    return 0;
  }

  enum : int { SORT_FAST = 0, SORT_EXACT = 1, SORT_CLOSED_FORM = 2 };
  static constexpr bool SORT_CLOSED = !SIM && (KS_SORT_CLOSED == 2 || (KS_SORT_CLOSED == 1 && LEAN));
  static constexpr bool CLOSED_SHIFT = KS_CLOSED_SHIFT && SORT_CLOSED && LEAN && RT > 0;
  int64_t shiftDiff = 0;
  __device__ __forceinline__ int sort_claims(int n, int pos, int& npos) {
    int tlo = n, thi = -1, pivot = -1;
    bool done = false;
    PH_BEGIN(tsc);
#ifdef KS_PHASE_STATS
    if (n <= 12) XPH_COUNT(SS_SORTS_LE12);
    else if (n < 50) XPH_COUNT(SS_SORTS_LT50);
#endif
    bool closed = false, shifted = false;
    npos = -1;
    if (n > 12) {
      int hint = 0, pv = 0, ts = -1;
      if constexpr (CLOSED_SHIFT) ts = closed_crossing<RM>(n, pos, s_ptpl, s_phead, hint, pv);
      else pv = w_choose_pivot(0, n, hint);
      if (hint == 1) {
        pivot = pv;
        if (ts >= 0) {
          tlo = pos;
          thi = npos = pos + ts;
          done = closed = shifted = true;
        }
        if constexpr (SORT_CLOSED && !CLOSED_SHIFT) {
          if (pos >= 0 && n >= 50 && pos + 1 < n) {
            const int t = closed_move(n, pos);
            if (t >= 0) {
              tlo = pos;
              thi = npos = pos + t;
              done = closed = true;
            }
          }
        }
      }
    }
    if (!closed) {
      const uint32_t g = KS_SORT_OUTLINE && LEAN && !SIM ? claim_sort_general_out(s_okey, s_order, n, pivot)
                                                          : claim_sort_general<LEAN && !SIM>(s_okey, s_order, n, pivot);
      tlo = (int)(g & 0x7fff);
      thi = (int)(g >> 15 & 0x7fff) - 1;
      done = g >> 30 & 1;
    }
    wsync();
#ifdef KS_PHASE_STATS
    if (shifted) {
      int diff = 0;
      for (int j = tlo + lane(); j <= thi; j += kWave) {
        const int c = s_order[j];
        const bool inl = c < pl.KL;
        bool ne = s_ptpl[j] != (inl ? tplv(lc.tpl[c]) : W.c_tpl[c]);
        for (int r = 0; r < R(); r++) {
          const int64_t i = (int64_t)c * R() + r;
          ne = ne || s_phead[(int64_t)j * R() + r] != (inl ? lc.max[i] - lc.req[i] : gc.max[i] - gc.req[i]);
        }
        diff += ne ? 1 : 0;
      }
      shiftDiff += wred_add(diff);
    }
#endif
    if (!shifted) {
      for (int j = tlo + lane(); j <= thi; j += kWave) {
        const int c = s_order[j];
        const bool inl = c < pl.KL;
        s_ptpl[j] = inl ? tplv(lc.tpl[c]) : W.c_tpl[c];
        for (int r = 0; r < R(); r++) {
          const int64_t i = (int64_t)c * R() + r;
          s_phead[(int64_t)j * R() + r] = inl ? lc.max[i] - lc.req[i] : gc.max[i] - gc.req[i];
        }
      }
      wsync();
    }
    algbytes += (int64_t)(thi - tlo + 1) * (8 + 16 * R());
#ifdef KS_PHASE_STATS
    if (closed) XPH_END(tsc, SS_SORT_CLOSED);
    else if (done) XPH_END(tsc, SS_SORT_FAST);
    else {
      XPH_END(tsc, SS_SORT_EXACT);
      const uint64_t dt = __builtin_amdgcn_s_memtime() - tsc;
      ecyc[0] += n <= 12 ? dt : 0;
      ecyc[1] += n > 12 && n < 50 ? dt : 0;
      ecyc[2] += n >= 50 ? dt : 0;
    }
#endif
    return closed ? SORT_CLOSED_FORM : done ? SORT_FAST : SORT_EXACT;
  }

  __device__ __forceinline__ int run_count_below(int p, int n, int K) const {
    int t = 0;
    for (int base = p + 1; base < n; base += 4 * kWave) {
      uint64_t m[4];
#pragma unroll
      for (int u = 0; u < 4; u++) {
        const int q = base + u * kWave + lane();
        m[u] = wballot(q < n && s_okey[q] < K);
      }
      bool end = false;
#pragma unroll
      for (int u = 0; u < 4; u++) {
        t += end ? 0 : popc64(m[u]);
        end = end || m[u] != ~0ull;
      }
      if (end) break;
    }
    return t;
  }
  __device__ __forceinline__ void run_materialise(int pos0, int p, int K) {
    pis_move(pos0, p);
    s_okey[p] = K;
    wsync();
    if (p == pos0) return;
    for (int j = pos0 + lane(); j <= p; j += kWave) {
      const int c = s_order[j];
      const bool inl = c < pl.KL;
      s_ptpl[j] = inl ? tplv(lc.tpl[c]) : W.c_tpl[c];
      for (int r = 0; r < R(); r++) {
        const int64_t i = (int64_t)c * R() + r;
        s_phead[(int64_t)j * R() + r] = inl ? lc.max[i] - lc.req[i] : gc.max[i] - gc.req[i];
      }
    }
    wsync();
  }

  template <class PR>
  __device__ __forceinline__ double worst_price(int it, PR rs, bool spot, bool od) const {
    const int b = D.it_off_beg[it], e = D.it_off_beg[it + 1];
    for (int pass = 0; pass < 2; pass++) {
      if (!(pass == 0 ? spot : od)) continue;
      const int want = pass == 0 ? d.spotBit : d.odBit;
      bool any = false;
      double w = 0;
      for (int o = b; o < e; o++)
        if (D.off_ct[o] == want && rs_member(L, rs, d.zoneKey, D.off_zone[o])) {
          const double pr = D.off_price[o];
          if (!any || pr > w) w = pr;
          any = true;
        }
      if (any) return w;
    }
    return __DBL_MAX__;
  }
  template <class PI, class PO, class PR>
  __device__ __forceinline__ int price_filter(PI in, PO out, int t, PR rs, bool spot, bool od, double price) const {
    const int tb = s_tbeg[t], nIT = s_tbeg[t + 1] - tb;
    int cnt = 0;
    for (int base = 0; base < nIT; base += kWave) {
      const int pos = base + lane();
      bool keep = pos < nIT && ((in[pos >> 5] >> (pos & 31)) & 1u);
      if (keep) keep = worst_price(D.tpl_its[tb + pos], rs, spot, od) < price;
      const uint64_t m = wballot(keep);
      if (lane() == 0) {
        out[base >> 5] = (uint32_t)m;
        if ((base >> 5) + 1 < d.TW) out[(base >> 5) + 1] = (uint32_t)(m >> 32);
      }
      cnt += __popcll(m);
    }
    return cnt;
  }
  __device__ __forceinline__ void sim_record(int P, int nclaims, int hostCtr, bool allSched, int err, bool anyPushed,
                                             bool anyRelaxed) {
    if (anyPushed) {
      hbm_release();
      bool bad = false;
      for (int i = lane(); i < P; i += kWave)
        bad |= ld_sc1(W.pod_status + i) == ST_FAILED && !(D.pod_flags[W.pod_map[i]] & PF_PROVISIONABLE);
      allSched = allSched && wballot(bad) == 0;
    }
    int32_t KS_G* rec = W.rec;
    const int TW = d.TW;
    int32_t KS_G* o_opt = rec + RF_HDR;
    int32_t KS_G* o_price = o_opt + TW;
    int32_t KS_G* o_same = o_price + TW;
    for (int i = lane(); i < 3 * TW; i += kWave) o_opt[i] = 0;
    int flags = (allSched ? RB_ALL_SCHEDULED : 0) | (anyRelaxed ? RB_RELAXED : 0), tpl = -1, host = -1, nopt = 0,
        nprice = 0, nsame = 0;
    int action = CA_NOOP;
    if (nclaims > 0 && err == KE_OK) {
      const int c = uni(s_order[0]);
      const bool inl = c < pl.KL;
      tpl = inl ? tplv(uni(lc.tpl[c])) : uni(W.c_tpl[c]);
      host = W.c_host[c];
      const uint32_t KS_G* crs = W.c_rs + (int64_t)c * d.RSW;
      wsync();
      for (int i = lane(); i < TW; i += kWave) o_opt[i] = inl ? lc.rem[(int64_t)c * TW + i] : gc.rem[(int64_t)c * TW + i];
      rec[RF_CLAIM] = c;
      {
        int cc = 0;
        for (int i = lane(); i < TW; i += kWave) cc += __popc(inl ? lc.rem[(int64_t)c * TW + i] : gc.rem[(int64_t)c * TW + i]);
        nopt = wred_add(cc);
      }
      const bool spot = rs_member(L, crs, d.ctKey, d.spotBit), od = rs_member(L, crs, d.ctKey, d.odBit);
      flags |= (spot ? RB_HAS_SPOT : 0) | (od ? RB_HAS_OD : 0);
      if (allSched && nclaims == 1) {
        if (W.cflags & CF_PRICE_ERR) {
          action = CA_ERROR;
// ... 269 lines not shown
    KsDev D, const KsWork* works, Plan pl, int nmw, int n, int stride) {
  extern __shared__ __attribute__((aligned(16))) char smem_mixed[];
  char KS_L* base = (char KS_L*)smem_mixed;
  if ((int)blockIdx.x < nmw) {
    solve_body<RT, true, true, false, true, true>(D, works, pl, (int)blockIdx.x, base);
  } else {
    const int wv = (int)(threadIdx.x >> 6);
    const int s = nmw + ((int)blockIdx.x - nmw) * kMwWaves + wv;
    if (s < n) solve_body<RT, true, true, false, true, false>(D, works, pl, s, base + (size_t)wv * stride);
  }
}

template <bool SIM, bool TOPO>
hipError_t launch_family(const KsDev& D, const KsWork* works_dev, int n, const Plan& pl, hipStream_t st) {
#define KS_LAUNCH(RT_, TL_, LEAN_)                                                                                 \
  do {                                                                                                             \
    route_note(Route{SIM ? (TOPO ? KR_SIMS_TOPO : KR_SIMS) : (TOPO ? KR_SOLVE_TOPO : KR_SOLVE), RT_, TL_, LEAN_, n, 0}); \
    hipLaunchKernelGGL((k_solve<RT_, TL_, SIM, TOPO, LEAN_>), dim3(n), dim3(kWave), pl.lds, st, D, works_dev, pl); \
  } while (0)
  if (n <= 0) return hipSuccess;
  const bool tl = pl.talloc != 0;
  const bool lean = !TOPO && D.d.lean && tl;
  switch (D.d.R) {
    case 3: if (lean) KS_LAUNCH(3, true, !TOPO); else if (tl) KS_LAUNCH(3, true, false); else KS_LAUNCH(3, false, false); break;
    case 4: if (lean) KS_LAUNCH(4, true, !TOPO); else if (tl) KS_LAUNCH(4, true, false); else KS_LAUNCH(4, false, false); break;
    default: if (tl) KS_LAUNCH(0, true, false); else KS_LAUNCH(0, false, false); break;
  }
#undef KS_LAUNCH
  return hipGetLastError();
}
using FamilyFn = hipError_t (*)(const KsDev&, const KsWork*, int, const Plan&, hipStream_t);
hipError_t launch_solve_plain(const KsDev& D, const KsWork* w, int n, const Plan& pl, hipStream_t st);
hipError_t launch_solve_topo(const KsDev& D, const KsWork* w, int n, const Plan& pl, hipStream_t st);
hipError_t launch_sims_plain(const KsDev& D, const KsWork* w, int n, const Plan& pl, hipStream_t st);
hipError_t launch_sims_topo(const KsDev& D, const KsWork* w, int n, const Plan& pl, hipStream_t st);
hipError_t launch_sims_mw(const KsDev& D, const KsWork* w, int n, const Plan& pl, hipStream_t st);
hipError_t launch_sims_mixed(const KsDev& D, const KsWork* w, int n, int nmw, const Plan& pl, hipStream_t st);

#if KS_TU == 1
hipError_t launch_solve_topo(const KsDev& D, const KsWork* w, int n, const Plan& pl, hipStream_t st) {
  return launch_family<false, true>(D, w, n, pl, st);
}
#elif KS_TU == 2
hipError_t launch_sims_plain(const KsDev& D, const KsWork* w, int n, const Plan& pl, hipStream_t st) {
  return launch_family<true, false>(D, w, n, pl, st);
}
hipError_t launch_sims_mixed(const KsDev& D, const KsWork* w, int n, int nmw, const Plan& pl, hipStream_t st) {
  if (n <= 0) return hipSuccess;
  const size_t stride = (pl.lds + 15) & ~(size_t)15;
  const size_t lds = std::max(pl.lds + kMwBytes, (size_t)kMwWaves * stride);
  if (D.d.G || !D.d.lean || !pl.talloc || D.d.N <= 0 || lds > 160 * 1024) return hipErrorNotSupported;
  const int grid = nmw + (n - nmw + kMwWaves - 1) / kMwWaves;
  const dim3 blk(kMwWaves * kWave);
  if (D.d.R == 3 || D.d.R == 4) route_note(Route{KR_SIMS_MIXED, D.d.R, 1, 1, n, nmw});
  switch (D.d.R) {
    case 3: hipLaunchKernelGGL((k_sim_mixed<3>), dim3(grid), blk, lds, st, D, w, pl, nmw, n, (int)stride); break;
    case 4: hipLaunchKernelGGL((k_sim_mixed<4>), dim3(grid), blk, lds, st, D, w, pl, nmw, n, (int)stride); break;
    default: return hipErrorNotSupported;
  }
  return hipGetLastError();
}
hipError_t launch_sims_mw(const KsDev& D, const KsWork* w, int n, const Plan& pl, hipStream_t st) {
  if (n <= 0) return hipSuccess;
  if (D.d.G || !D.d.lean || !pl.talloc || D.d.N <= 0 || pl.lds + kMwBytes > 160 * 1024) return hipErrorNotSupported;
  const dim3 blk(kMwWaves * kWave);
  if (D.d.R == 3 || D.d.R == 4) route_note(Route{KR_SIMS_MW, D.d.R, 1, 1, n, 0});
  switch (D.d.R) {
    case 3: hipLaunchKernelGGL((k_solve<3, true, true, false, true, true>), dim3(n), blk, pl.lds + kMwBytes, st, D, w, pl); break;
    case 4: hipLaunchKernelGGL((k_solve<4, true, true, false, true, true>), dim3(n), blk, pl.lds + kMwBytes, st, D, w, pl); break;
    default: return hipErrorNotSupported;
  }
  return hipGetLastError();
}
#elif KS_TU == 3
hipError_t launch_sims_topo(const KsDev& D, const KsWork* w, int n, const Plan& pl, hipStream_t st) {
  return launch_family<true, true>(D, w, n, pl, st);
}
#else
hipError_t launch_solve_plain(const KsDev& D, const KsWork* w, int n, const Plan& pl, hipStream_t st) {
  return launch_family<false, false>(D, w, n, pl, st);
}

static Plan make_plan_live(const KsDims& d, size_t budget, bool sim, int wideKO, bool live, int frontTotal);
Plan make_plan(const KsDims& d, size_t budget, bool sim, int wideKO, int frontTotal) {
  const bool rt = d.R == 3 || d.R == 4;
  if (sim || !rt) return make_plan_live(d, budget, sim, wideKO, false, frontTotal);
  if (d.lean) {
    const Plan lean = make_plan_live(d, budget, sim, wideKO, false, frontTotal);
    if (lean.talloc) return lean;
  }
  return make_plan_live(d, budget, sim, wideKO, true, frontTotal);
}

static Plan make_plan_live(const KsDims& d, size_t budget, bool sim, int wideKO, bool live, int frontTotal) {
  auto r16 = [](size_t b) { return (b + 15) & ~(size_t)15; };
  Plan pl{};
  const size_t R = d.R, TW = d.TW, tot = d.totalTplIts;
  const size_t fixed = r16(sizeof(KeyMeta) * d.NK) + r16(4 * (size_t)(d.NTPL + 1)) + r16(8 * (size_t)(d.NPOOL + 1) * R) +
                       2 * r16(4 * (size_t)d.RSW) + 5 * r16(4 * TW + 8) + 16 * 16 + (d.volAny ? 48 : 0) +
                       (KS_TPL_MEMO && !sim && d.lean ? r16(4 * (size_t)tpl_memo_words((int)R, (int)TW)) : 0) +
                       (KS_RUN_FRONT && KS_CLAIM_RUNS && !sim && d.lean ? r16(4 * (size_t)(d.NTPL + 1)) + r16(4 * (size_t)frontTotal) : 0) +
                       (sim ? 4 * r16(4 * (size_t)((d.N + 31) / 32)) : d.fnOn ? r16(4 * (size_t)((d.N + 31) / 32)) : 0) +
                       (d.G ? r16(4 * (size_t)d.G * TGM_WORDS) + r16(4 * (size_t)d.G) + 2 * r16(4 * (size_t)d.RSW) +
                                  (d.GMW > 1 ? r16(8 * (size_t)GS_N * d.GMW) : 0) +
                                  (sim ? r16(4 * (size_t)((d.tgCntWords - d.tgSmall + 31) / 32)) + 4 * kTdwKeys * kTdw : 0)
                              : 0);
  const size_t posB = 16 + 8 * R;
  const size_t clmB = 16 + 16 * R + 4 * TW + 4 * R;
  const size_t slack = 10 * 16;
  const size_t tallocB = r16(8 * tot * R);
  const size_t tsortB = r16(8 * tot * R) + r16(4 * tot * R);
  size_t avail = budget > fixed + slack ? budget - fixed - slack : 0;
  pl.tcl = d.G ? d.tgSmall : 0;
  if (d.G && !sim && 4 * (size_t)d.tgCntWords <= avail / 4) pl.tcl = d.tgCntWords;
  const size_t tclB = r16(4 * (size_t)pl.tcl);
  avail = avail > tclB ? avail - tclB : 0;
  const size_t tdWords = (size_t)d.TK * (size_t)d.N;
  pl.tdl = d.G && !sim && tdWords > 0 && 4 * tdWords <= avail / 4 ? (int32_t)tdWords : 0;
  const size_t tdlB = r16(4 * (size_t)pl.tdl);
  avail = avail > tdlB ? avail - tdlB : 0;
  pl.livl = live && d.N > 0 && !d.negReq && !d.tgUnlab && 4 * (size_t)d.N <= avail / 4 ? d.N : 0;
  const size_t livB = r16(4 * (size_t)pl.livl);
  avail = avail > livB ? avail - livB : 0;
  const size_t tablesB = tallocB + (d.negReq ? 0 : tsortB);
  pl.talloc = (wideKO < 2 && tablesB + 64 * (posB + clmB) <= avail) ? 1 : 0;
  pl.tsort = pl.talloc && !d.negReq;
  if (pl.talloc) avail -= tablesB;
  const size_t tmaskB = tpl_mask_bytes(d.NTPL, (int)TW);
  pl.tmask = (KS_TPL_MASKS && !sim && d.lean && pl.talloc && tpl_mask_fits(avail, d.NTPL, (int)TW, posB, clmB)) ? 1 : 0;
  if (pl.tmask) avail -= tmaskB;
  const size_t kAll = avail / (posB + clmB);
  size_t ko, kl;
  if (kAll >= (size_t)d.Kcap) {
    ko = kl = d.Kcap;
  } else if (wideKO) {
    kl = std::min<size_t>(64, kAll);
    ko = std::min((size_t)d.Kcap, (avail - kl * clmB) / posB);
  } else {
    ko = std::min((size_t)d.Kcap, std::max(kAll, avail / 2 / posB));
    kl = std::min(ko, (avail - ko * posB) / clmB);
  }
  pl.KO = (int)ko;
  pl.KL = (int)kl;
  pl.lds = fixed + tclB + tdlB + livB + 3 * r16(4 * ko) + r16(8 * ko * R) + 2 * r16(4 * kl) + 2 * r16(8 * kl * R) + r16(4 * kl * TW) +
           r16(4 * kl * R) + (pl.tsort ? tsortB : 0) + (pl.talloc ? tallocB : 0) + (pl.tmask ? tmaskB : 0);
  return pl;
}

int run_fuse_build() { return KS_RUN_FUSE; }
int tpl_masks_build() { return KS_TPL_MASKS; }
int log_runs_build() { return KS_LOG_RUNS && KS_CLAIM_RUNS; }
int sort_leaf_build() { return KS_SORT_LEAF && !KS_SORT_LANE0; }
int closed_shift_build() { return KS_CLOSED_SHIFT && KS_SORT_CLOSED; }

template <int R>
__global__ __attribute__((amdgpu_flat_work_group_size(64, 64))) void k_claim_sort_probe(
    int32_t* keys, int32_t* order, int n, int mode, int pos, const int32_t* ctpl, const int64_t* chead, int32_t* ptpl,
    int64_t* phead, int32_t* how) {
  extern __shared__ __attribute__((aligned(16))) char smem_probe[];
  char KS_L* sp = (char KS_L*)smem_probe;
  const size_t n4 = (4 * (size_t)n + 15) & ~(size_t)15;
  ClaimSort cs;
  LI64 s_phead = (LI64)sp;
  cs.s_okey = (LI32)(sp + 8 * (size_t)n * R);
  cs.s_order = (LI32)(sp + 8 * (size_t)n * R + n4);
  LI32 s_ptpl = (LI32)(sp + 8 * (size_t)n * R + 2 * n4);
  auto gather = [&](int lo, int hi) {
    for (int j = lo + lane(); j <= hi; j += kWave) {
      const int c = cs.s_order[j];
      s_ptpl[j] = ctpl[c];
      for (int r = 0; r < R; r++) s_phead[(int64_t)j * R + r] = chead[(int64_t)c * R + r];
    }
    wsync();
  };
  for (int j = lane(); j < n; j += kWave) {
    cs.s_okey[j] = keys[j];
    cs.s_order[j] = order[j];
  }
  wsync();
  gather(0, n - 1);
  if (mode == 0) pos = -1;
  int tlo = n, thi = -1, pivot = -1, res = 1;
  bool closed = false;
  if (n > 12) {
    int hint = 0, pv = 0, ts = -1;
    if (KS_CLOSED_SHIFT && KS_SORT_CLOSED) ts = cs.closed_crossing<R>(n, pos, s_ptpl, s_phead, hint, pv);
    else pv = cs.w_choose_pivot(0, n, hint);
    if (hint == 1) {
      pivot = pv;
      if (ts >= 0) closed = true;
      else if (KS_SORT_CLOSED && !KS_CLOSED_SHIFT && pos >= 0 && n >= 50 && pos + 1 < n) {
        const int t = cs.closed_move(n, pos);
        if (t >= 0) {
          closed = true;
          tlo = pos;
          thi = pos + t;
        }
      }
    }
  }
  if (closed) res = 2;
  else {
    const uint32_t g = claim_sort_general<true>(cs.s_okey, cs.s_order, n, pivot);
    tlo = (int)(g & 0x7fff);
    thi = (int)(g >> 15 & 0x7fff) - 1;
    res = g >> 30 & 1 ? 0 : 1;
  }
  wsync();
  gather(tlo, thi);
  for (int j = lane(); j < n; j += kWave) {
    keys[j] = cs.s_okey[j];
    order[j] = cs.s_order[j];
    ptpl[j] = s_ptpl[j];
    for (int r = 0; r < R; r++) phead[(int64_t)j * R + r] = s_phead[(int64_t)j * R + r];
  }
  how[lane()] = res;
}
hipError_t claim_sort_probe(int32_t* keys, int32_t* order, int n, int mode, int pos, int R, const int32_t* ctpl,
                            const int64_t* chead, int32_t* ptpl, int64_t* phead, int32_t* how, hipStream_t st) {
  if (n < 0 || n > kProbeMaxN || (R != 3 && R != 4)) return hipErrorInvalidValue;
  const size_t lds = 8 * (size_t)n * R + 3 * ((4 * (size_t)n + 15) & ~(size_t)15) + 16;
  if (R == 3) hipLaunchKernelGGL((k_claim_sort_probe<3>), dim3(1), dim3(kWave), lds, st, keys, order, n, mode, pos, ctpl, chead, ptpl, phead, how);
  else hipLaunchKernelGGL((k_claim_sort_probe<4>), dim3(1), dim3(kWave), lds, st, keys, order, n, mode, pos, ctpl, chead, ptpl, phead, how);
  return hipGetLastError();
}

void launch_feasibility(const KsDev& D, hipStream_t st) {
  const int rows = D.d.S * D.d.NTPL;
  if (D.d.TW <= 32) {
    const int blocks = std::min(2048, (rows + 7) / 8);
    hipLaunchKernelGGL(k_feasibility<32>, dim3(blocks), dim3(256), 0, st, D);
  } else {
    const int blocks = std::min(2048, (rows + 3) / 4);
    hipLaunchKernelGGL(k_feasibility<64>, dim3(blocks), dim3(256), 0, st, D);
  }
}

void launch_feasibility_nodes(const KsDev& D, hipStream_t st) {
  const int nbx = (D.d.N + 255) / 256;
  hipLaunchKernelGGL(k_feasibility_nodes, dim3(D.d.FNR * nbx), dim3(256), 0, st, D, nbx);
}

hipError_t queue_sort(const KsDev& D, uint64_t* keys, int32_t* vals, void* temp, size_t tempBytes, int32_t* out,
                      hipStream_t st);
hipError_t sim_run_lengths(const int32_t* podmap, const int32_t* entry_sim, const int64_t* pod_req, const uint64_t* pod_s0,
                           const int32_t* pod_flags, int R, int n, uint64_t* words, int32_t* run_len, hipStream_t st,
                           bool strict);

hipError_t launch_solve(const KsDev& D, const KsWork* works_dev, int nrep, const Plan& pl, int32_t* qorder,
                        uint64_t* skeys, int32_t* svals, void* stemp, size_t stempBytes, hipStream_t st,
                        hipEvent_t mid, const int32_t* fixed_order, hipEvent_t* feas, int32_t* run_len,
                        uint64_t* run_words, hipEvent_t post) {
  if (pl.lds > 160 * 1024) return hipErrorInvalidValue;
  if (!fixed_order) {
    hipError_t e = queue_sort(D, skeys, svals, stemp, stempBytes, qorder, st);
    if (e != hipSuccess) return e;
  }
  if (D.d.lean && run_len && run_words) {
    hipError_t e = sim_run_lengths(fixed_order ? fixed_order : qorder, nullptr, D.pod_req, D.pod_s0, D.pod_flags, D.d.R,
                                   D.d.P, run_words, run_len, st, true);
    if (e != hipSuccess) return e;
  }
  if (D.d.fmOn) {
    if (feas) (void)hipEventRecord(feas[0], st);
    launch_feasibility(D, st);
    if (feas) (void)hipEventRecord(feas[1], st);
  }
  if (D.d.fnOn) {
    if (feas) (void)hipEventRecord(feas[2], st);
    launch_feasibility_nodes(D, st);
    if (feas) (void)hipEventRecord(feas[3], st);
  }
  hipLaunchKernelGGL(k_init, dim3(512), dim3(256), 0, st, D, works_dev, nrep,
                     fixed_order ? fixed_order : (const int32_t*)qorder);
  if (mid) (void)hipEventRecord(mid, st);
  hipError_t e = (D.d.G ? launch_solve_topo : launch_solve_plain)(D, works_dev, nrep, pl, st);
  if (post) (void)hipEventRecord(post, st);
  const bool leanRoute = !D.d.G && D.d.lean && pl.talloc && (D.d.R == 3 || D.d.R == 4);
  if (e == hipSuccess && log_runs_build() && leanRoute && nrep > 0 && D.d.P > 0) {
    const int bx = std::min(256, std::max(1, (D.d.P + 255) / 256)), by = std::min(nrep, 1024);
    hipLaunchKernelGGL(k_log_expand, dim3(bx, by), dim3(256), 0, st, works_dev, nrep,
                       fixed_order ? fixed_order : (const int32_t*)qorder, D.d.P);
    e = hipGetLastError();
  }
  return e;
}

hipError_t launch_sims(const KsDev& D, const KsWork* works_dev, int nsims, const Plan& pl, hipStream_t st) {
  if (pl.lds > 160 * 1024) return hipErrorInvalidValue;
  if (nsims <= 0) return hipSuccess;
  if (D.d.fmOn) launch_feasibility(D, st);
  if (D.d.fnOn) launch_feasibility_nodes(D, st);
  return (D.d.G ? launch_sims_topo : launch_sims_plain)(D, works_dev, nsims, pl, st);
}
bool sims_mw_supported(const KsDev& D, const Plan& pl) {
  return !D.d.G && D.d.lean && pl.talloc && D.d.N > 0 && pl.lds + kMwBytes <= 160 * 1024 && (D.d.R == 3 || D.d.R == 4);
}
hipError_t launch_sims_split(const KsDev& D, const KsWork* works_dev, int nsims, int nmw, const Plan& pl, hipStream_t st,
                             hipStream_t st2, hipEvent_t fork, hipEvent_t join) {
  if (nmw <= 0 || !sims_mw_supported(D, pl)) return launch_sims(D, works_dev, nsims, pl, st);
  if (pl.lds > 160 * 1024) return hipErrorInvalidValue;
  if (D.d.fmOn) launch_feasibility(D, st);
  if (D.d.fnOn) launch_feasibility_nodes(D, st);
  const hipError_t em = launch_sims_mixed(D, works_dev, nsims, nmw, pl, st);
  if (em != hipErrorNotSupported) return em;
  hipError_t e = hipEventRecord(fork, st);
  if (e == hipSuccess) e = hipStreamWaitEvent(st2, fork, 0);
  if (e == hipSuccess) e = launch_sims_mw(D, works_dev, nmw, pl, st2);
  if (e == hipSuccess && nsims > nmw) e = launch_sims_plain(D, works_dev + nmw, nsims - nmw, pl, st);
  if (e == hipSuccess) e = hipEventRecord(join, st2);
  if (e == hipSuccess) e = hipStreamWaitEvent(st, join, 0);
  return e;
}
#endif

}
```

### karpenter-sigs_amd/csrc/ks_solve_body.inc

```
  constexpr int RM = Solver<RT, TL, SIM, TOPO, LEAN>::RM;
#ifdef KS_FORCE_UNIFORM
  constexpr bool FORCEU = SIM || !LEAN;
#else
  constexpr bool FORCEU = SIM && LEAN;
#endif
  auto U = [](bool x) { return FORCEU ? ub(x) : x; };
  auto UI = [](int x) { return FORCEU ? uni(x) : x; };
  KS_BODY_SMEM_DECL
  const KsWork KS_C& W = KS_BODY_WORK;
  const KsDims& d = D.d;
  Solver<RT, TL, SIM, TOPO, LEAN> S(D, W, pl);
  const int R = S.R();
  char KS_L* sp = smem;
  auto take = [&](size_t bytes) { char KS_L* r = sp; sp += (bytes + 15) & ~(size_t)15; return r; };
  KeyMeta KS_L* s_keys = (KeyMeta KS_L*)take(sizeof(KeyMeta) * d.NK);
  S.s_order = (LI32)take(4 * (size_t)pl.KO);
  S.s_okey = (LI32)take(4 * (size_t)pl.KO);
  S.s_ptpl = (LI32)take(4 * (size_t)pl.KO);
  S.s_phead = (LI64)take(8 * (size_t)pl.KO * R);
  S.lc.tpl = (LI32)take(4 * (size_t)pl.KL);
  S.lc.req = (LI64)take(8 * (size_t)pl.KL * R);
  S.lc.max = (LI64)take(8 * (size_t)pl.KL * R);
  S.lc.rem = (LU32)take(4 * (size_t)pl.KL * d.TW);
  S.lc.thr = (LI32)take(4 * (size_t)pl.KL * R);
// ... 1019 lines not shown
                    srt = inl ? S.template commit_bulk<true>(c, pos, nclaims, kk, podk, req, nthr, kcnt)
                              : S.template commit_bulk<false>(c, pos, nclaims, kk, podk, req, nthr, kcnt);
                    if constexpr (SORTC) dpos = srt ? -1 : pos;
                    S.algbytes = ab0 + credit;
                    SXPH_END(S, tbk, SS_BULK);
                    PH_BEGIN(tlg);
                    if (wi + k <= wn) {
                      const int src = wi + lane() < kWave ? wi + lane() : kWave - 1;
                      S.log_batch(k, __shfl(w.p, src), c, nlog);
                    } else if constexpr (Solver<RT, TL, SIM, TOPO, LEAN>::LOG_RUNS) {
                      S.log_run_record(k, qhead, c, nlog);
                      SYPH_END(S, tlg, YS_LOG_STORE);
                    } else if constexpr (KS_LOG_AHEAD) {
                      for (int b = 0; b < k; b += 4 * kWave) {
                        int pv[4];
#pragma unroll
                        for (int u = 0; u < 4; u++) {
                          const int e = b + u * kWave + lane();
                          int pos = qhead + (e < k ? e : k - 1);
                          pos = pos >= P ? pos - P : pos;
                          pv[u] = W.queue[pos];
                        }
#pragma unroll
                        for (int u = 0; u < 4; u++) {
                          const int left = k - b - u * kWave;
                          if (left > 0) S.log_batch(left < kWave ? left : kWave, pv[u], c, nlog);
                        }
                      }
                    } else {
                      for (int b = 0; b < k; b += kWave) {
                        int pos = qhead + b + lane();
                        pos = pos >= P ? pos - P : pos;
                        PH_BEGIN(tyq);
                        const int pv = b + lane() < k ? W.queue[pos] : 0;
                        PH_WAIT_LOADS();
                        SYPH_END(S, tyq, YS_LOG_LOAD);
                        PH_BEGIN(tyb);
                        S.log_batch(k - b < kWave ? k - b : kWave, pv, c, nlog);
                        SYPH_END(S, tyb, YS_LOG_STORE);
                      }
                    }
                    SXPH_END(S, tlg, SS_LOG);
                    qhead += k;
                    if (qhead >= P) qhead -= P;
                    qlen -= k;
                    pops += k;
                    wi += k;
                    if (wi > wn) wi = wn;
                    runs++;
                    runPods += k;
                  }
                }
              }
            }
          } else {
            fullFails++;
            stepFF++;
            const int t = inl ? S.tplv(uni(S.lc.tpl[c])) : uni(W.c_tpl[c]);
            if (inl) S.template recompute_max<true>(c, S.lc.rem + (int64_t)c * d.TW, t, jj);
            else S.template recompute_max<false>(c, S.gc.rem + (int64_t)c * d.TW, t, jj);
          }
          PH_END(t5, 5);
        }
      }
    }
    if (!U(placed)) {
      PH_BEGIN(t6);
      const int r = U(simNoClaim) ? S.sim_template_calls(hostCtr)
                                  : UI(S.try_templates(p, s, sflags, toltpl, pod, nclaims, nlog, hostCtr, srt));
      PH_END(t6, 6);
      nclaims = UI(nclaims);
      hostCtr = UI(hostCtr);
      srt = U(srt);
      dpos = -1;
      if (r < 0) { err = KE_CLAIM_CAP; break; }
      if (r == 1) placed = true;
      if (r == 2) {
        W.pod_status[p] = ST_SCHEDULED;
        placed = true;
      }
    }
    if (U(placed)) {
      if (SIM && rdl(w.st, wi - 1) == ST_FAILED) W.pod_status[p] = ST_SCHEDULED;
      continue;
    }
    if constexpr (LEAN && !SIM) {
      if (d.dupUids) {
        err = KE_LEAN_EXIT;
        break;
      }
    }
    if (SIM && ident) S.sim_queue_init(P);
    const int s0 = D.pod_state0[g], ns = D.pod_nstate[g];
    const bool relaxed = U(s - s0 + 1 < ns);
    W.pod_status[p] = ST_FAILED;
    W.pod_fstate[p] = s;
    if (relaxed) W.pod_state[p] = s + 1;
    if (relaxed) epoch++;
    anyRelaxed = anyRelaxed || relaxed;
    if (TOPO && relaxed) S.topo_activate_state(s + 1, nclaims, hostCtr);
    int tail = qhead + qlen;
    if (tail >= P) tail -= P;
    W.queue[tail] = p;
    qlen++;
    pushed = true;
    ident = false;
    if (!relaxed) W.last_len[uid] = ((uint64_t)epoch << 32) | (uint32_t)qlen;
  }
  if constexpr (MWK) {
    mw_post(MW_EXIT, 0, pod, 0, 0, 0);
    mw_barrier();
    bool hall = true;
    int64_t hab = 0;
#pragma unroll
    for (int q = 1; q < kMwWaves; q++) {
      hall = hall && mb[MB_ALL + q] != 0;
      hab += (int64_t)mb_ld64(mb, MB_AB + 2 * q);
    }
    allSched = allSched && ub(hall);
    S.algbytes += uni64(hab);
  }
  S.log_flush(nlog);
  for (int i = lane(); i < nclaims; i += kWave) W.order[i] = S.s_order[i];
  const int kl = nclaims < pl.KL ? nclaims : pl.KL;
  for (int i = lane(); i < kl * R; i += kWave) W.c_req[i] = S.lc.req[i];
  for (int i = lane(); i < kl * d.TW; i += kWave) W.c_rem[i] = S.lc.rem[i];
  if (lane() == 0) {
    W.counters[CT_NCLAIMS] = nclaims;
    W.counters[CT_NLOG] = nlog;
    W.counters[CT_HOSTCTR] = hostCtr;
    W.counters[CT_ERROR] = err;
    W.counters[CT_POPS] = pops;
    W.counters[CT_ALGBYTES] = S.algbytes;
    W.counters[CT_SORTS] = sorts;
    W.counters[CT_SORT_SLOW] = slow;
    W.counters[CT_CLAIM_FULL] = fulls;
    W.counters[CT_CLAIM_QUICK_FAIL] = fullFails;
    W.counters[CT_WINDOWS] = windows;
    W.counters[CT_RUNS] = runs;
    W.counters[CT_RUN_PODS] = runPods;
    W.counters[CT_SORT_EXACT] = exact;
    W.counters[CT_RUN_CROSS] = cross;
    W.counters[CT_RUN_CROSS_STOPS] = crossStops;
    W.counters[CT_RUN_CROSS_LOST] = crossLost;
    W.counters[CT_SORT_CLOSED] = sortsClosed;
    W.counters[CT_TPL_MEMO_HITS] = S.memoHits;
    W.counters[CT_RUN_CAP_FRONT] = S.capFront;
    W.counters[CT_RUN_CAP_FULL] = S.capFull;
    W.counters[CT_RUN_CROSS_CLOSED] = crossClosed;
    W.counters[CT_RUN_MOVES] = runMoves;
    W.counters[CT_TPL_MASK_FILLS] = S.maskFills;
    W.counters[CT_TPL_MASK_HITS] = S.maskHits;
    W.counters[CT_RUN_RECS] = S.runRecs;
#ifdef KS_PHASE_STATS
    for (int i = 0; i < 7; i++) W.counters[CT_CYC_POP + i] = (int64_t)cyc[i];
    W.counters[CT_CYC_TOTAL] = (int64_t)(__builtin_amdgcn_s_memtime() - tstart);
    W.counters[CT_CYC_NCOMMIT] = (int64_t)cyc[7];
    for (int i = 0; i < 4; i++) W.counters[CT_CYC_SUB + i] = (int64_t)S.scyc[i];
    for (int i = 0; i < 8; i++) W.counters[CT_FINE + i] = (int64_t)fcyc[i];
    for (int i = 0; i < 12; i++) W.counters[CT_STEP + i] = (int64_t)S.xcyc[i];
    for (int i = 0; i < 3; i++) W.counters[CT_CYC_EXACT_BY_N + i] = (int64_t)S.ecyc[i];
    W.counters[CT_CLOSED_SHIFT_DIFF] = S.shiftDiff;
    for (int i = 0; i < 6; i++) W.counters[CT_CYC_SPLIT + i] = (int64_t)S.ycyc[i];
#endif
  }
  if constexpr (SIM) S.sim_record(P, nclaims, hostCtr, allSched, err, !ident, anyRelaxed);
```

### karpenter-sigs_amd/csrc/ks_sort_probe.h

```cpp
#pragma once
#include <stddef.h>
#include <stdint.h>

#include "ks_gosort.h"
#include "ks_problem.h"

namespace ks {

inline const char* sort_probe_check(int mode, int pos, int n, int R, const int32_t* keys, const int32_t* order,
                                    const int32_t* claim_tpl, const int64_t* claim_head, const int32_t* ptpl,
                                    const int64_t* phead) {
  if (n < 0 || n > kProbeMaxN) return "n must be 0 .. kProbeMaxN";
  if (R != 3 && R != 4) return "R must be 3 or 4";
  if (mode != 0 && mode != 1) return "mode must be 0 or 1";
  if (mode == 1 && (pos < 0 || pos >= n)) return "mode 1 needs 0 <= pos < n";
  if (n > 0 && (!keys || !order || !claim_tpl || !claim_head || !ptpl || !phead)) return "null argument";
  for (int j = 0; j < n; j++)
    if (order[j] < 0 || order[j] >= n) return "order holds claim ids 0 .. n - 1";
  return nullptr;
}

inline void sort_probe_host(int n, int R, int32_t* keys, int32_t* order, const int32_t* claim_tpl,
                            const int64_t* claim_head, int32_t* ptpl, int64_t* phead) {
  GoSortExact g{GoSort{keys, order}};
  g.run(n);
  for (int j = 0; j < n; j++) {
    const int c = order[j];
    ptpl[j] = claim_tpl[c];
    for (int r = 0; r < R; r++) phead[(size_t)j * R + r] = claim_head[(size_t)c * R + r];
  }
}

}
```

### karpenter-sigs_amd/karpenter_amd/scheduler.py

```python
import ctypes
import json
import os

_HERE = os.path.dirname(os.path.abspath(__file__))
_VARIANTS = {"stats": "libkarpenter_amd_stats.so", "asan": "libkarpenter_amd_asan.so", "tsan": "libkarpenter_amd_tsan.so"}
_VARIANT = os.environ.get("KS_LIB_VARIANT", "")
_LIB_PATH = os.path.join(_HERE, _VARIANTS.get(_VARIANT, "libkarpenter_amd_%s.so" % _VARIANT if _VARIANT else "libkarpenter_amd.so"))
_lib = None

KS_ERRORS = {-1: "KS_ERR_PARSE", -2: "KS_ERR_UNSUPPORTED", -3: "KS_ERR_CAPACITY", -4: "KS_ERR_HIP",
             -5: "KS_ERR_INTERNAL", -6: "KS_ERR_ARG"}


class KsError(RuntimeError):
    def __init__(self, code, msg):
        super().__init__("%s: %s" % (KS_ERRORS.get(code, code), msg))
        self.code = code


class _Opts(ctypes.Structure):
    _fields_ = [("device", ctypes.c_int), ("simulation_mode", ctypes.c_int), ("replicas", ctypes.c_int),
                ("timing_only", ctypes.c_int), ("lds_budget", ctypes.c_int),
                ("reserved", ctypes.c_int * 3)]


class _Clock(ctypes.Structure):
    _fields_ = [("multi_timeout_s", ctypes.c_double), ("single_timeout_s", ctypes.c_double),
                ("sim_seconds", ctypes.c_double)]


def library_path():
    return _LIB_PATH


def lib():
    global _lib
    if _lib is not None:
        return _lib
    if not os.path.exists(_LIB_PATH):
        raise KsError(-4, "libkarpenter_amd.so not built (%s); run __graft_entry__.build()" % _LIB_PATH)
    l = ctypes.CDLL(_LIB_PATH)
    vp = ctypes.c_void_p
    l.ks_problem_create.argtypes = [ctypes.c_char_p, ctypes.c_size_t, ctypes.POINTER(vp)]
    l.ks_problem_inspect.argtypes = [ctypes.c_char_p, ctypes.c_size_t, ctypes.POINTER(vp)]
    l.ks_problem_free.argtypes = [vp]
    l.ks_solve.argtypes = [vp, ctypes.POINTER(_Opts), ctypes.POINTER(vp)]
    l.ks_results_free.argtypes = [vp]
    l.ks_results_json.argtypes = [vp, ctypes.POINTER(vp)]
    l.ks_results_kernel_ms.argtypes = [vp]
    l.ks_results_kernel_ms.restype = ctypes.c_double
    l.ks_results_solve_kernel_ms.argtypes = [vp]
    l.ks_results_solve_kernel_ms.restype = ctypes.c_double
    l.ks_results_algorithmic_bytes.argtypes = [vp]
    l.ks_results_algorithmic_bytes.restype = ctypes.c_double
    l.ks_results_feasibility_ms.argtypes = [vp]
    l.ks_results_feasibility_ms.restype = ctypes.c_double
    l.ks_results_feasibility_bytes.argtypes = [vp]
    l.ks_results_feasibility_bytes.restype = ctypes.c_double
    l.ks_results_node_feasibility_ms.argtypes = [vp]
    l.ks_results_node_feasibility_ms.restype = ctypes.c_double
    l.ks_results_node_feasibility_bytes.argtypes = [vp]
    l.ks_results_node_feasibility_bytes.restype = ctypes.c_double
    l.ks_cluster_state.argtypes = [ctypes.c_char_p, ctypes.c_size_t, ctypes.POINTER(vp)]
    l.ks_free.argtypes = [vp]
    l.ks_problem_save.argtypes = [vp, ctypes.POINTER(vp), ctypes.POINTER(ctypes.c_size_t)]
    l.ks_problem_create_binary.argtypes = [ctypes.c_char_p, ctypes.c_size_t, ctypes.POINTER(vp)]
    l.ks_snapshot_check.argtypes = [ctypes.c_char_p, ctypes.c_size_t, ctypes.POINTER(ctypes.c_size_t)]
    l.ks_problem_encode_binary.argtypes = [ctypes.c_char_p, ctypes.c_size_t, ctypes.POINTER(vp),
                                           ctypes.POINTER(ctypes.c_size_t)]
    l.ks_problem_check_binary.argtypes = [ctypes.c_char_p, ctypes.c_size_t]
    l.ks_problem_feasibility_rows.argtypes = [vp, ctypes.c_int, ctypes.POINTER(vp), ctypes.POINTER(vp),
                                              ctypes.POINTER(ctypes.c_size_t)]
    l.ks_problem_queue_inputs.argtypes = [ctypes.c_char_p, ctypes.c_size_t, ctypes.POINTER(vp)]
    l.ks_problem_queue_readback.argtypes = [vp, ctypes.POINTER(vp), ctypes.POINTER(vp), ctypes.POINTER(ctypes.c_size_t),
                                            ctypes.POINTER(ctypes.c_int)]
    l.ks_rec_headers_run.argtypes = [vp, vp, ctypes.c_int, ctypes.c_int, vp, ctypes.c_int, vp, vp, ctypes.POINTER(vp),
                                     ctypes.POINTER(vp)]
    l.ks_cons_save.argtypes = [vp, ctypes.POINTER(vp), ctypes.POINTER(ctypes.c_size_t)]
    l.ks_cons_create_binary.argtypes = [ctypes.c_char_p, ctypes.c_size_t, ctypes.POINTER(vp)]
    l.ks_last_error.restype = ctypes.c_char_p
    l.ks_build_info.restype = ctypes.c_char_p
    _lib = l
    return l


def _check(rc):
    if rc != 0:
        raise KsError(rc, lib().ks_last_error().decode())


def _take_str(ptr):
    s = ctypes.cast(ptr, ctypes.c_char_p).value.decode()
    lib().ks_free(ptr)
    return s


def _encode(snapshot):
    return (snapshot if isinstance(snapshot, str) else json.dumps(snapshot)).encode()


def _records_buffer(records):
    if (isinstance(records, memoryview) and isinstance(records.obj, ctypes.Array)
            and records.nbytes == ctypes.sizeof(records.obj)):
        return records.obj
    return ctypes.create_string_buffer(bytes(records), len(records))


def inspect(snapshot):
    b = _encode(snapshot)
    out = ctypes.c_void_p()
    _check(lib().ks_problem_inspect(b, len(b), ctypes.byref(out)))
    return json.loads(_take_str(out))


def queue_inputs(snapshot):
    b = _encode(snapshot)
    out = ctypes.c_void_p()
    _check(lib().ks_problem_queue_inputs(b, len(b), ctypes.byref(out)))
    return json.loads(_take_str(out))


def rec_headers_meta():
    meta = ctypes.c_void_p()
    _check(lib().ks_rec_headers_run(None, None, 0, 0, None, 0, None, None, None, ctypes.byref(meta)))
    return json.loads(_take_str(meta))


def rec_headers_verdicts(records, tw, tpl_beg):
    import numpy as np

    flat = np.ascontiguousarray(np.array(records, dtype=np.int32))
    ns = np.array([len(records)], dtype=np.int32)
    tb = np.array(tpl_beg, dtype=np.int32)
    verdicts = ctypes.c_void_p()
    _check(lib().ks_rec_headers_run(flat.ctypes.data, ns.ctypes.data, 1, tw, tb.ctypes.data, len(tb) - 1, None, None,
                                    ctypes.byref(verdicts), None))
    return json.loads(_take_str(verdicts))[0]


def rec_headers_run(passes, tw, tpl_beg):
    import numpy as np

    flat = np.ascontiguousarray(np.array([r for batch in passes for r in batch], dtype=np.int32))
    ns = np.array([len(batch) for batch in passes], dtype=np.int32)
    tb = np.array(tpl_beg, dtype=np.int32)
    rf_hdr = rec_headers_meta()["RF_HDR"]
    assert flat.ndim == 2 and flat.shape[1] == rf_hdr + 3 * tw
    hdr = np.zeros(int(ns.sum()) * rf_hdr, dtype=np.int32)
    status = np.zeros(2 * len(passes), dtype=np.uint64)
    verdicts = ctypes.c_void_p()
    _check(lib().ks_rec_headers_run(flat.ctypes.data, ns.ctypes.data, len(passes), tw, tb.ctypes.data, len(tb) - 1,
                                    hdr.ctypes.data, status.ctypes.data, ctypes.byref(verdicts), None))
    verdicts = json.loads(_take_str(verdicts))
    out, at = [], 0
    for i, n in enumerate(ns):
        out.append(([int(x) for x in hdr[at:at + int(n) * rf_hdr]], [int(status[2 * i]), int(status[2 * i + 1])],
                    verdicts[i]))
        at += int(n) * rf_hdr
    return out


def claim_sort_probe(keys, order, claim_tpl, claim_head, mode=0, pos=-1, device=0):
    import numpy as np

    k = np.array(keys, dtype=np.int32)
    o = np.array(order, dtype=np.int32)
    ct = np.ascontiguousarray(claim_tpl, dtype=np.int32)
    ch = np.ascontiguousarray(claim_head, dtype=np.int64)
    n = len(k)
    assert len(o) == n and len(ct) == n and ch.ndim == 2 and ch.shape[0] == n
    r = ch.shape[1]
    pt = np.zeros(n, dtype=np.int32)
    ph = np.zeros((n, r), dtype=np.int64)
    how = ctypes.c_int(-1)
    lib().ks_claim_sort_probe.argtypes = [ctypes.c_int] * 5 + [ctypes.c_void_p] * 6 + [ctypes.POINTER(ctypes.c_int)]
    _check(lib().ks_claim_sort_probe(device, mode, pos, n, r, k.ctypes.data, o.ctypes.data, ct.ctypes.data,
                                     ch.ctypes.data, pt.ctypes.data, ph.ctypes.data, ctypes.byref(how)))
    return k, o, pt, ph, how.value


def cluster_state(cluster):
    b = _encode(cluster)
    out = ctypes.c_void_p()
    _check(lib().ks_cluster_state(b, len(b), ctypes.byref(out)))
    return json.loads(_take_str(out))


class Results:

    def __init__(self, doc, kernel_ms, alg_bytes, solve_kernel_ms=0.0):
        self.doc = doc
        self.new_nodeclaims = doc["newNodeClaims"]
        self.existing_nodes = doc["existingNodes"]
        self.pod_errors = {int(k): v for k, v in doc["podErrors"].items()}
        self.stats = doc.get("stats", {})
        self.kernel_ms = kernel_ms
        self.solve_kernel_ms = solve_kernel_ms
        self.algorithmic_bytes = alg_bytes
        self.feasibility_ms = 0.0
        self.feasibility_bytes = 0.0
        self.node_feasibility_ms = 0.0
        self.node_feasibility_bytes = 0.0

    def canonical(self):
        d = dict(self.doc)
        d.pop("stats", None)
        return d


class _Requirement(ctypes.Structure):
    _fields_ = [("key", ctypes.c_char_p), ("op", ctypes.c_char_p), ("n_values", ctypes.c_int),
                ("values", ctypes.POINTER(ctypes.c_char_p)), ("has_gt", ctypes.c_int), ("has_lt", ctypes.c_int),
                ("gt", ctypes.c_int64), ("lt", ctypes.c_int64)]


_accessors_bound = False


def _bind_accessors(l):
    global _accessors_bound
    if _accessors_bound:
        return
    vp, ip = ctypes.c_void_p, ctypes.POINTER(ctypes.c_int)
    i32pp = ctypes.POINTER(ctypes.POINTER(ctypes.c_int32))
    strpp = ctypes.POINTER(ctypes.POINTER(ctypes.c_char_p))
    l.ks_results_num_new_nodeclaims.argtypes = [vp]
    l.ks_results_nodeclaim.argtypes = [vp, ctypes.c_int, ip, i32pp, ip, i32pp, ip]
    l.ks_results_nodeclaim_requests.argtypes = [vp, ctypes.c_int, ip, strpp, strpp]
    l.ks_results_nodeclaim_requirements.argtypes = [vp, ctypes.c_int, ip, ctypes.POINTER(ctypes.POINTER(_Requirement))]
    l.ks_results_num_existing_nodes.argtypes = [vp]
    l.ks_results_existing_node.argtypes = [vp, ctypes.c_int, ip, i32pp, ip]
    l.ks_results_num_pod_errors.argtypes = [vp]
    l.ks_results_pod_error.argtypes = [vp, ctypes.c_int, ip, ctypes.POINTER(ctypes.c_char_p)]
    _accessors_bound = True


class StructuredResults:

    def __init__(self, claims, nodes, errors, kernel_ms, solve_kernel_ms):
        self.new_nodeclaims = claims
        self.existing_nodes = nodes
        self.pod_errors = errors
        self.kernel_ms = kernel_ms
        self.solve_kernel_ms = solve_kernel_ms


def _read_structured(l, r):
    import numpy as np

    _bind_accessors(l)
    tpl, n1, n2 = ctypes.c_int(), ctypes.c_int(), ctypes.c_int()
    a1, a2 = ctypes.POINTER(ctypes.c_int32)(), ctypes.POINTER(ctypes.c_int32)()
    claims = []
    for i in range(l.ks_results_num_new_nodeclaims(r)):
        _check(l.ks_results_nodeclaim(r, i, ctypes.byref(tpl), ctypes.byref(a1), ctypes.byref(n1), ctypes.byref(a2),
                                      ctypes.byref(n2)))
        pods = np.ctypeslib.as_array(a1, (n1.value,)).copy() if n1.value else np.zeros(0, np.int32)
        its = np.ctypeslib.as_array(a2, (n2.value,)).copy() if n2.value else np.zeros(0, np.int32)
        names, qtys = ctypes.POINTER(ctypes.c_char_p)(), ctypes.POINTER(ctypes.c_char_p)()
        _check(l.ks_results_nodeclaim_requests(r, i, ctypes.byref(n1), ctypes.byref(names), ctypes.byref(qtys)))
        requests = {names[k].decode(): qtys[k].decode() for k in range(n1.value)}
        rq = ctypes.POINTER(_Requirement)()
        _check(l.ks_results_nodeclaim_requirements(r, i, ctypes.byref(n1), ctypes.byref(rq)))
        reqs = []
        for k in range(n1.value):
            x = rq[k]
            reqs.append((x.key.decode(), x.op.decode(), [x.values[v].decode() for v in range(x.n_values)],
                         x.gt if x.has_gt else None, x.lt if x.has_lt else None))
        claims.append({"template": tpl.value, "pods": pods, "instance_types": its, "requests": requests,
                       "requirements": reqs})
    nodes = []
    for i in range(l.ks_results_num_existing_nodes(r)):
        _check(l.ks_results_existing_node(r, i, ctypes.byref(n2), ctypes.byref(a1), ctypes.byref(n1)))
        pods = np.ctypeslib.as_array(a1, (n1.value,)).copy() if n1.value else np.zeros(0, np.int32)
        nodes.append((n2.value, pods))
    errors = {}
    msg = ctypes.c_char_p()
    for i in range(l.ks_results_num_pod_errors(r)):
        _check(l.ks_results_pod_error(r, i, ctypes.byref(n1), ctypes.byref(msg)))
        errors[n1.value] = msg.value.decode()
    return claims, nodes, errors


def _take_bytes(fn, handle):
    buf, n = ctypes.c_void_p(), ctypes.c_size_t()
    _check(fn(handle, ctypes.byref(buf), ctypes.byref(n)))
    try:
        return ctypes.string_at(buf, n.value)
    finally:
        lib().ks_free(buf)


def snapshot_check(snapshot):
    b = _encode(snapshot)
    n = ctypes.c_size_t()
    _check(lib().ks_snapshot_check(b, len(b), ctypes.byref(n)))
    return n.value


def encode_binary(snapshot):
    b = _encode(snapshot)
    buf, n = ctypes.c_void_p(), ctypes.c_size_t()
    _check(lib().ks_problem_encode_binary(b, len(b), ctypes.byref(buf), ctypes.byref(n)))
    try:
        return ctypes.string_at(buf, n.value)
    finally:
        lib().ks_free(buf)


def check_binary(blob):
    blob = bytes(blob)
    _check(lib().ks_problem_check_binary(blob, len(blob)))


class Scheduler:

    def __init__(self, snapshot, _binary=None):
        h = ctypes.c_void_p()
        if _binary is not None:
            _check(lib().ks_problem_create_binary(_binary, len(_binary), ctypes.byref(h)))
        else:
            b = _encode(snapshot)
            _check(lib().ks_problem_create(b, len(b), ctypes.byref(h)))
        self._h = h

    @classmethod
    def from_binary(cls, blob):
# ... 346 lines not shown
```

Baseline: 7.734 million pods/s.

## Sort small claim lists in wave registers instead of LDS

Adds a register-resident pdqsort (SortRegsT) that keeps up to 64 claim keys and values in VGPRs across the wavefront. It uses readlane, ballot and ds_permute in place of LDS-based ClaimSort, and falls back to the LDS sort on budget or stack overflow. This targets LDS traffic and sync overhead in the outlined general claim sort on LEAN non-sim kernels. A packed single-pass radix sort for queue keys is also added but disabled by default. Costs are extra registers, cross-lane permute overhead, and new counters and a probe path.

```diff
diff --git a/include/karpenter_amd.h b/include/karpenter_amd.h
--- a/include/karpenter_amd.h
+++ b/include/karpenter_amd.h
@@ -45,6 +45,9 @@
 int ks_problem_queue_readback(ks_problem* p, int32_t** order, int32_t** run_len, size_t* n, int* device_sorted);
 int ks_claim_sort_probe(int device, int mode, int pos, int n, int R, int32_t* keys, int32_t* order,
                         const int32_t* claim_tpl, const int64_t* claim_head, int32_t* ptpl, int64_t* phead, int* how);
+int ks_claim_sort_probe_path(int device, int mode, int pos, int n, int R, int32_t* keys, int32_t* order,
+                             const int32_t* claim_tpl, const int64_t* claim_head, int32_t* ptpl, int64_t* phead,
+                             int* how, int* path);
 int ks_rec_headers_run(const int32_t* records, const int32_t* pass_ns, int n_passes, int TW, const int32_t* tpl_beg,
                        int ntpl, int32_t* headers, uint64_t* status, char** verdicts_json, char** meta_json);
 
diff --git a/karpenter-sigs_amd/csrc/ks_capi.cpp b/karpenter-sigs_amd/csrc/ks_capi.cpp
--- a/karpenter-sigs_amd/csrc/ks_capi.cpp
+++ b/karpenter-sigs_amd/csrc/ks_capi.cpp
@@ -1126,7 +1126,8 @@
   pareto_fronts(d, h.tab.tpl_it_beg, h.tab.tpl_its, h.tab.it_alloc, frontBeg, frontPos);
   o += ",\"runFuse\":" + std::to_string(run_fuse_build()) + ",\"sortLeaf\":" + std::to_string(sort_leaf_build()) +
        ",\"closedShift\":" + std::to_string(closed_shift_build()) + ",\"tplMasks\":" + std::to_string(tpl_masks_build()) +
-       ",\"logRuns\":" + std::to_string(log_runs_build()) + ",\"paretoFronts\":[";
+       ",\"logRuns\":" + std::to_string(log_runs_build()) + ",\"sortRegs\":" + std::to_string(sort_regs_build()) +
+       ",\"sortRegsN64\":" + std::to_string(sort_regs_n64_build()) + ",\"queuePacked\":" + std::to_string(queue_packed_build()) + ",\"paretoFronts\":[";
   for (int t = 0; t < d.NTPL; t++) {
     o += t ? ",[" : "[";
     for (int i = frontBeg[(size_t)t]; i < frontBeg[(size_t)t + 1]; i++)
@@ -1309,9 +1310,20 @@
 
 int ks_claim_sort_probe(int device, int mode, int pos, int n, int R, int32_t* keys, int32_t* order,
                         const int32_t* claim_tpl, const int64_t* claim_head, int32_t* ptpl, int64_t* phead, int* how) {
+  return ks_claim_sort_probe_path(device, mode, pos, n, R, keys, order, claim_tpl, claim_head, ptpl, phead, how, nullptr);
+}
+int ks_claim_sort_probe_path(int device, int mode, int pos, int n, int R, int32_t* keys, int32_t* order,
+                             const int32_t* claim_tpl, const int64_t* claim_head, int32_t* ptpl, int64_t* phead,
+                             int* how, int* path) {
   API_TRY
   if (const char* bad = sort_probe_check(mode, pos, n, R, keys, order, claim_tpl, claim_head, ptpl, phead))
     throw KsError(KS_ERR_ARG, bad);
+  if (path) *path = 0;
+  if (device == -2 || device == -3) {
+    const int h = sort_probe_model(n, R, keys, order, claim_tpl, claim_head, ptpl, phead, device == -2, path);
+    if (how) *how = h;
+    return KS_OK;
+  }
   if (device < 0) {
     sort_probe_host(n, R, keys, order, claim_tpl, claim_head, ptpl, phead);
     if (how) *how = 1;
@@ -1347,16 +1359,17 @@
     HIPCHK(hipMemcpyAsync(b.chead, claim_head, 8 * (size_t)n * R, hipMemcpyHostToDevice, b.stream));
   }
   HIPCHK(claim_sort_probe(b.keys, b.order, n, mode, pos, R, b.ctpl, b.chead, b.ptpl, b.phead, b.how, b.stream));
-  int32_t h = -1;
+  int32_t h[2] = {-1, 0};
   if (n > 0) {
     HIPCHK(hipMemcpyAsync(keys, b.keys, 4 * (size_t)n, hipMemcpyDeviceToHost, b.stream));
     HIPCHK(hipMemcpyAsync(order, b.order, 4 * (size_t)n, hipMemcpyDeviceToHost, b.stream));
     HIPCHK(hipMemcpyAsync(ptpl, b.ptpl, 4 * (size_t)n, hipMemcpyDeviceToHost, b.stream));
     HIPCHK(hipMemcpyAsync(phead, b.phead, 8 * (size_t)n * R, hipMemcpyDeviceToHost, b.stream));
   }
-  HIPCHK(hipMemcpyAsync(&h, b.how, 4, hipMemcpyDeviceToHost, b.stream));
+  HIPCHK(hipMemcpyAsync(h, b.how, 8, hipMemcpyDeviceToHost, b.stream));
   HIPCHK(hipStreamSynchronize(b.stream));
-  if (how) *how = h;
+  if (how) *how = h[0];
+  if (path) *path = h[1];
   return KS_OK;
   API_CATCH
 }
@@ -1520,7 +1533,7 @@
                                 "cycRunCap", "cycCross", "cycBulk", "cycLog", "cycTplDerive", "cycTplStore",
                                 "cycTplMax", "runCapFront", "runCapFull", "runCrossClosed", "runMoves",
                                 "cycSortExactLe12", "cycSortExactLt50", "cycSortExactGe50", "closedShiftDiff",
-                                "tplMaskFills", "tplMaskHits", "runRecs",
+                                "tplMaskFills", "tplMaskHits", "runRecs", "sortsRegs", "sortRegsBail", "sortRegsOver",
                                 "cycTplCand", "cycTplFeas", "cycTplFilter", "cycTplThr", "cycLogLoad", "cycLogStore"};
   static_assert(sizeof(names) / sizeof(names[0]) == CT_NCOUNTERS, "one name per counter");
   for (int i = 0; i < CT_NCOUNTERS; i++) o += std::string(i ? "," : "") + "\"" + names[i] + "\":" + std::to_string(r->counters[i]);
diff --git a/karpenter-sigs_amd/csrc/ks_problem.h b/karpenter-sigs_amd/csrc/ks_problem.h
--- a/karpenter-sigs_amd/csrc/ks_problem.h
+++ b/karpenter-sigs_amd/csrc/ks_problem.h
@@ -288,6 +288,9 @@
   CT_TPL_MASK_FILLS,
   CT_TPL_MASK_HITS,
   CT_RUN_RECS,
+  CT_SORT_REGS,
+  CT_SORT_REGS_BAIL,
+  CT_SORT_REGS_OVER,
   CT_CYC_SPLIT,
   CT_CYC_SPLIT_END = CT_CYC_SPLIT + 6,
   CT_NCOUNTERS = CT_CYC_SPLIT_END
diff --git a/karpenter-sigs_amd/csrc/ks_queue.hip b/karpenter-sigs_amd/csrc/ks_queue.hip
--- a/karpenter-sigs_amd/csrc/ks_queue.hip
+++ b/karpenter-sigs_amd/csrc/ks_queue.hip
@@ -1,4 +1,8 @@
 #include <hip/hip_runtime.h>
+
+#ifndef KS_QUEUE_PACKED
+#define KS_QUEUE_PACKED 0
+#endif
 
 #include <hipcub/hipcub.hpp>
 
@@ -14,6 +18,24 @@
   keys[i] = (uint64_t)(sortkey[(int64_t)p * 4 + comp] - minv);
   vals[i] = p;
 }
+
+struct QPack {
+  int64_t minv[4];
+  int32_t shift[4];
+  int32_t bits[4];
+};
+__global__ void k_qkeys_packed(const int64_t* sortkey, QPack q, uint64_t* keys, int32_t* vals, int n) {
+  const int i = blockIdx.x * blockDim.x + threadIdx.x;
+  if (i >= n) return;
+  uint64_t k = 0;
+#pragma unroll
+  for (int c = 0; c < 4; c++)
+    if (q.bits[c] > 0) k |= (uint64_t)(sortkey[(int64_t)i * 4 + c] - q.minv[c]) << q.shift[c];
+  keys[i] = k;
+  vals[i] = i;
+}
+
+int queue_packed_build() { return KS_QUEUE_PACKED; }
 
 __global__ void k_iota(int32_t* v, int n) {
   const int i = blockIdx.x * blockDim.x + threadIdx.x;
@@ -33,6 +55,20 @@
   const int n = d.P;
   if (n == 0) return hipSuccess;
   const int blocks = (n + 255) / 256;
+  const int total = d.skBits[0] + d.skBits[1] + d.skBits[2] + d.skBits[3];
+  if (KS_QUEUE_PACKED && total > 0 && total <= 64) {
+    QPack q;
+    int below = 0;
+    for (int comp = 3; comp >= 0; comp--) {
+      q.minv[comp] = d.skMin[comp];
+      q.bits[comp] = d.skBits[comp];
+      q.shift[comp] = below;
+      below += d.skBits[comp];
+    }
+    hipLaunchKernelGGL(k_qkeys_packed, dim3(blocks), dim3(256), 0, st, D.pod_sortkey, q, keys, vals, n);
+    size_t tb = tempBytes;
+    return hipcub::DeviceRadixSort::SortPairs(temp, tb, keys, keys + n, vals, out, n, 0, total, st);
+  }
   const int32_t* cur = nullptr;
   int buf = 0;
   for (int comp = 3; comp >= 0; comp--) {
diff --git a/karpenter-sigs_amd/csrc/ks_runtime.h b/karpenter-sigs_amd/csrc/ks_runtime.h
--- a/karpenter-sigs_amd/csrc/ks_runtime.h
+++ b/karpenter-sigs_amd/csrc/ks_runtime.h
@@ -26,6 +26,9 @@
 int closed_shift_build();
 int tpl_masks_build();
 int log_runs_build();
+int sort_regs_build();
+int sort_regs_n64_build();
+int queue_packed_build();
 hipError_t claim_sort_probe(int32_t* keys, int32_t* order, int n, int mode, int pos, int R, const int32_t* ctpl,
                             const int64_t* chead, int32_t* ptpl, int64_t* phead, int32_t* how, hipStream_t st);
 Plan make_plan(const KsDims& d, size_t budget, bool sim = false, int wideKO = 0, int frontTotal = 0);
diff --git a/karpenter-sigs_amd/csrc/ks_solve.hip b/karpenter-sigs_amd/csrc/ks_solve.hip
--- a/karpenter-sigs_amd/csrc/ks_solve.hip
+++ b/karpenter-sigs_amd/csrc/ks_solve.hip
@@ -39,6 +39,12 @@
 #ifndef KS_SORT_OUTLINE
 #define KS_SORT_OUTLINE 1
 #endif
+#ifndef KS_SORT_REGS
+#define KS_SORT_REGS 1
+#endif
+#ifndef KS_SORT_REGS_N64
+#define KS_SORT_REGS_N64 1
+#endif
 #ifndef KS_TPL_MEMO
 #define KS_TPL_MEMO 1
 #endif
@@ -55,6 +61,7 @@
 #include "ks_gosort.h"
 #include "ks_problem.h"
 #include "ks_reqset.h"
+#include "ks_sort_regs.h"
 #include "ks_tplmask.h"
 
 namespace ks {
@@ -897,8 +904,39 @@
     }
   }
 };
-template <bool LEAF>
+struct SortRegsWaveOps {
+  using Vec = int;
+  template <class F> static __device__ __forceinline__ void each(F f) { f(lane()); }
+  static __device__ __forceinline__ int& at(Vec& v, int) { return v; }
+  static __device__ __forceinline__ int get(const Vec& v, int) { return v; }
+  static __device__ __forceinline__ int rdl(Vec v, int l) { return __builtin_amdgcn_readlane(v, l); }
+  template <class F> static __device__ __forceinline__ uint64_t ballot(F p) { return wballot(p(lane())); }
+  template <class F> static __device__ __forceinline__ Vec gather(Vec v, F src) {
+    return __builtin_amdgcn_ds_bpermute(src(lane()) * 4, v);
+  }
+  template <class F> static __device__ __forceinline__ Vec scatter(Vec v, F dst) {
+    return __builtin_amdgcn_ds_permute(dst(lane()) * 4, v);
+  }
+};
+template <bool LEAF, bool REGS = false>
 static __device__ __forceinline__ uint32_t claim_sort_general(LI32 okey, LI32 order, int n, int pivot) {
+  if constexpr (REGS && KS_SORT_REGS != 0) {
+    n = uni(n);
+    pivot = uni(pivot);
+    if (n <= (KS_SORT_REGS_N64 ? 64 : kSortRegsMax)) {
+      SortRegsT<SortRegsWaveOps, !KS_SORT_REGS_N64> rs;
+      rs.load(n, [&](int p) { return okey[p]; }, [&](int p) { return order[p]; });
+      const uint32_t g = rs.general(pivot);
+      if (g != 0) {
+        rs.store([&](int p, int k, int v) {
+          okey[p] = k;
+          order[p] = v;
+        });
+        wsync();
+        return g;
+      }
+    }
+  }
   ClaimSort cs;
   cs.s_order = order;
   cs.s_okey = okey;
@@ -920,7 +958,7 @@
   return (uint32_t)tlo | (uint32_t)(thi + 1) << 15 | (uint32_t)done << 30;
 }
 static __device__ __noinline__ uint32_t claim_sort_general_out(LI32 okey, LI32 order, int n, int pivot) {
-  return claim_sort_general<true>(okey, order, n, pivot);
+  return claim_sort_general<true, true>(okey, order, n, pivot);
 }
 
 template <int RT, bool TL, bool SIM, bool TOPO, bool LEAN>
@@ -2410,6 +2448,8 @@
   enum : int { SORT_FAST = 0, SORT_EXACT = 1, SORT_CLOSED_FORM = 2 };
   static constexpr bool SORT_CLOSED = !SIM && (KS_SORT_CLOSED == 2 || (KS_SORT_CLOSED == 1 && LEAN));
   static constexpr bool CLOSED_SHIFT = KS_CLOSED_SHIFT && SORT_CLOSED && LEAN && RT > 0;
+  static constexpr bool SORT_REGS = KS_SORT_REGS != 0 && KS_SORT_OUTLINE && LEAN && !SIM;
+  int sortsRegs = 0, sortRegsOver = 0, sortRegsBail = 0;
   int64_t shiftDiff = 0;
   __device__ __forceinline__ int sort_claims(int n, int pos, int& npos) {
     int tlo = n, thi = -1, pivot = -1;
@@ -2450,6 +2490,12 @@
       tlo = (int)(g & 0x7fff);
       thi = (int)(g >> 15 & 0x7fff) - 1;
       done = g >> 30 & 1;
+      if constexpr (SORT_REGS) {
+        const bool over = n > (KS_SORT_REGS_N64 ? 64 : kSortRegsMax);
+        sortsRegs += (int)(g >> 31);
+        sortRegsOver += over ? 1 : 0;
+        sortRegsBail += !over && !(g >> 31) ? 1 : 0;
+      }
     }
     wsync();
 #ifdef KS_PHASE_STATS
@@ -3025,6 +3071,8 @@
 int log_runs_build() { return KS_LOG_RUNS && KS_CLAIM_RUNS; }
 int sort_leaf_build() { return KS_SORT_LEAF && !KS_SORT_LANE0; }
 int closed_shift_build() { return KS_CLOSED_SHIFT && KS_SORT_CLOSED; }
+int sort_regs_build() { return KS_SORT_REGS != 0 && KS_SORT_OUTLINE; }
+int sort_regs_n64_build() { return sort_regs_build() && KS_SORT_REGS_N64; }
 
 template <int R>
 __global__ __attribute__((amdgpu_flat_work_group_size(64, 64))) void k_claim_sort_probe(
@@ -3072,12 +3120,14 @@
       }
     }
   }
+  int path = 0;
   if (closed) res = 2;
   else {
-    const uint32_t g = claim_sort_general<true>(cs.s_okey, cs.s_order, n, pivot);
+    const uint32_t g = claim_sort_general<true, true>(cs.s_okey, cs.s_order, n, pivot);
     tlo = (int)(g & 0x7fff);
     thi = (int)(g >> 15 & 0x7fff) - 1;
     res = g >> 30 & 1 ? 0 : 1;
+    path = g & kSortRegsDone ? 1 : KS_SORT_REGS == 0 ? 0 : n > (KS_SORT_REGS_N64 ? 64 : kSortRegsMax) ? 3 : 2;
   }
   wsync();
   gather(tlo, thi);
@@ -3087,7 +3137,7 @@
     ptpl[j] = s_ptpl[j];
     for (int r = 0; r < R; r++) phead[(int64_t)j * R + r] = s_phead[(int64_t)j * R + r];
   }
-  how[lane()] = res;
+  how[lane()] = lane() == 1 ? path : res;
 }
 hipError_t claim_sort_probe(int32_t* keys, int32_t* order, int n, int mode, int pos, int R, const int32_t* ctpl,
                             const int64_t* chead, int32_t* ptpl, int64_t* phead, int32_t* how, hipStream_t st) {
diff --git a/karpenter-sigs_amd/csrc/ks_solve_body.inc b/karpenter-sigs_amd/csrc/ks_solve_body.inc
--- a/karpenter-sigs_amd/csrc/ks_solve_body.inc
+++ b/karpenter-sigs_amd/csrc/ks_solve_body.inc
@@ -1195,6 +1195,11 @@
     W.counters[CT_TPL_MASK_FILLS] = S.maskFills;
     W.counters[CT_TPL_MASK_HITS] = S.maskHits;
     W.counters[CT_RUN_RECS] = S.runRecs;
+    if constexpr (decltype(S)::SORT_REGS) {
+      W.counters[CT_SORT_REGS] = S.sortsRegs;
+      W.counters[CT_SORT_REGS_BAIL] = S.sortRegsBail;
+      W.counters[CT_SORT_REGS_OVER] = S.sortRegsOver;
+    }
 #ifdef KS_PHASE_STATS
     for (int i = 0; i < 7; i++) W.counters[CT_CYC_POP + i] = (int64_t)cyc[i];
     W.counters[CT_CYC_TOTAL] = (int64_t)(__builtin_amdgcn_s_memtime() - tstart);
diff --git a/karpenter-sigs_amd/csrc/ks_sort_probe.h b/karpenter-sigs_amd/csrc/ks_sort_probe.h
--- a/karpenter-sigs_amd/csrc/ks_sort_probe.h
+++ b/karpenter-sigs_amd/csrc/ks_sort_probe.h
@@ -4,6 +4,7 @@
 
 #include "ks_gosort.h"
 #include "ks_problem.h"
+#include "ks_sort_regs.h"
 
 namespace ks {
 
@@ -31,4 +32,15 @@
   }
 }
 
+inline int sort_probe_model(int n, int R, int32_t* keys, int32_t* order, const int32_t* claim_tpl,
+                            const int64_t* claim_head, int32_t* ptpl, int64_t* phead, bool two, int* path) {
+  const int how = sort_regs_model(n, keys, order, two, path);
+  for (int j = 0; j < n; j++) {
+    const int c = order[j];
+    ptpl[j] = claim_tpl[c];
+    for (int r = 0; r < R; r++) phead[(size_t)j * R + r] = claim_head[(size_t)c * R + r];
+  }
+  return how;
 }
+
+}
diff --git a/karpenter-sigs_amd/csrc/ks_sort_regs.h b/karpenter-sigs_amd/csrc/ks_sort_regs.h
--- /dev/null
+++ b/karpenter-sigs_amd/csrc/ks_sort_regs.h
@@ -0,0 +1,443 @@
+#pragma once
+#include <stdint.h>
+
+#include "ks_gosort.h"
+
+namespace ks {
+
+constexpr int kSortRegsMax = 128;
+
+KS_HD int choose_pivot_medians(int a, int b, int& hint, int k0, int k1, int k2, int k3, int k4, int k5, int k6, int k7,
+                               int k8) {
+  const int l = b - a;
+  int i = a + l / 4, j = a + l / 4 * 2, k = a + l / 4 * 3, swaps = 0;
+  if (l >= 8) {
+    auto median = [&](int ia, int ka, int ib, int kb, int ic, int kc, int& km) {
+      if (kb < ka) { swaps++; int t0 = ia; ia = ib; ib = t0; t0 = ka; ka = kb; kb = t0; }
+      if (kc < kb) { swaps++; int t0 = ib; ib = ic; ic = t0; t0 = kb; kb = kc; kc = t0; }
+      if (kb < ka) { swaps++; int t0 = ia; ia = ib; ib = t0; t0 = ka; ka = kb; kb = t0; }
+      km = kb;
+      return ib;
+    };
+    int ki = k1, kj = k4, kq = k7;
+    if (l >= 50) {
+      i = median(i - 1, k0, i, k1, i + 1, k2, ki);
+      j = median(j - 1, k3, j, k4, j + 1, k5, kj);
+      k = median(k - 1, k6, k, k7, k + 1, k8, kq);
+    }
+    int km = 0;
+    j = median(i, ki, j, kj, k, kq, km);
+  }
+  hint = swaps == 0 ? 1 : (swaps == 12 ? 2 : 0);
+  return j;
+}
+
+template <class W, bool TWO>
+struct SortRegsT {
+  using Vec = typename W::Vec;
+  Vec k0, v0, k1, v1;
+  int n = 0;
+  int bail = 0;
+  int breaks = 0;
+  int heaps = 0;
+
+  static KS_HD int popc(uint64_t m) { return __builtin_popcountll(m); }
+  static KS_HD int lowbit(uint64_t m) { return __builtin_ctzll(m); }
+  static KS_HD int highbit(uint64_t m) { return 63 - __builtin_clzll(m); }
+
+  template <class KF, class VF>
+  KS_HD void load(int n_, KF keyOf, VF valOf) {
+    n = n_;
+    W::each([&](int l) {
+      W::at(k0, l) = l < n ? keyOf(l) : INT32_MAX;
+      W::at(v0, l) = l < n ? valOf(l) : -1;
+      if (TWO) {
+        W::at(k1, l) = 64 + l < n ? keyOf(64 + l) : INT32_MAX;
+        W::at(v1, l) = 64 + l < n ? valOf(64 + l) : -1;
+      }
+    });
+  }
+  template <class PF>
+  KS_HD void store(PF put) const {
+    W::each([&](int l) {
+      if (l < n) put(l, W::get(k0, l), W::get(v0, l));
+      if (TWO && 64 + l < n) put(64 + l, W::get(k1, l), W::get(v1, l));
+    });
+  }
+
+  KS_HD int keyAt(int p) const {
+    const int lo = W::rdl(k0, p & 63);
+    if (!TWO) return lo;
+    const int hi = W::rdl(k1, p & 63);
+    return p < 64 ? lo : hi;
+  }
+  KS_HD int valAt(int p) const {
+    const int lo = W::rdl(v0, p & 63);
+    if (!TWO) return lo;
+    const int hi = W::rdl(v1, p & 63);
+    return p < 64 ? lo : hi;
+  }
+  KS_HD void setKey(int p, int k) {
+    W::each([&](int l) {
+      W::at(k0, l) = l == p ? k : W::get(k0, l);
+      if (TWO) W::at(k1, l) = 64 + l == p ? k : W::get(k1, l);
+    });
+  }
+  KS_HD void setVal(int p, int v) {
+    W::each([&](int l) {
+      W::at(v0, l) = l == p ? v : W::get(v0, l);
+      if (TWO) W::at(v1, l) = 64 + l == p ? v : W::get(v1, l);
+    });
+  }
+  KS_HD void swap(int i, int j) {
+    const int ki = keyAt(i), vi = valAt(i), kj = keyAt(j), vj = valAt(j);
+    W::each([&, i, j, ki, vi, kj, vj](int l) {
+      W::at(k0, l) = l == i ? kj : l == j ? ki : W::get(k0, l);
+      W::at(v0, l) = l == i ? vj : l == j ? vi : W::get(v0, l);
+      if (TWO) {
+        W::at(k1, l) = 64 + l == i ? kj : 64 + l == j ? ki : W::get(k1, l);
+        W::at(v1, l) = 64 + l == i ? vj : 64 + l == j ? vi : W::get(v1, l);
+      }
+    });
+  }
+  template <class F>
+  KS_HD void masks(F pred, uint64_t& m0, uint64_t& m1) const {
+    m0 = W::ballot([&](int l) { return pred(l, W::get(k0, l)); });
+    m1 = 0;
+    if (TWO) m1 = W::ballot([&](int l) { return pred(64 + l, W::get(k1, l)); });
+  }
+  template <class F>
+  KS_HD void pull(F src) {
+    const auto s0 = [&](int l) { return src(l) & 63; };
+    const Vec a0 = W::gather(k0, s0), b0 = W::gather(v0, s0);
+    if (!TWO) {
+      k0 = a0;
+      v0 = b0;
+      return;
+    }
+    const auto s1 = [&](int l) { return src(64 + l) & 63; };
+    const Vec a1 = W::gather(k1, s0), b1 = W::gather(v1, s0);
+    const Vec c0 = W::gather(k0, s1), d0 = W::gather(v0, s1), c1 = W::gather(k1, s1), d1 = W::gather(v1, s1);
+    W::each([&](int l) {
+      const bool lo0 = src(l) < 64, lo1 = src(64 + l) < 64;
+      W::at(k0, l) = lo0 ? W::get(a0, l) : W::get(a1, l);
+      W::at(v0, l) = lo0 ? W::get(b0, l) : W::get(b1, l);
+      W::at(k1, l) = lo1 ? W::get(c0, l) : W::get(c1, l);
+      W::at(v1, l) = lo1 ? W::get(d0, l) : W::get(d1, l);
+    });
+  }
+
+  KS_HD void move(int from, int to) {
+    if (from == to) return;
+    if (to < from) pull([=](int p) { return p == to ? from : (p > to && p <= from) ? p - 1 : p; });
+    else pull([=](int p) { return p == to ? from : (p >= from && p < to) ? p + 1 : p; });
+  }
+  KS_HD void reverse(int a, int b) {
+    pull([=](int p) { return p >= a && p < b ? a + b - 1 - p : p; });
+  }
+  KS_HD int descent(int from, int b) const {
+    const auto prev = [](int l) { return (l + 63) & 63; };
+    const Vec p0 = W::gather(k0, prev);
+    uint64_t m0 = W::ballot([&](int l) { return l >= from && l < b && W::get(k0, l) < W::get(p0, l); }), m1 = 0;
+    if (TWO) {
+      const Vec p1 = W::gather(k1, prev);
+      m1 = W::ballot([&](int l) {
+        return 64 + l >= from && 64 + l < b && W::get(k1, l) < (l == 0 ? W::get(p0, l) : W::get(p1, l));
+      });
+    }
+    return m0 ? lowbit(m0) : m1 ? 64 + lowbit(m1) : b;
+  }
+  KS_HD bool pis(int a, int b, int& tlo, int& thi) {
+    int i = a + 1;
+    for (int step = 0; step < 5; step++) {
+      i = descent(i, b);
+      if (i == b) return true;
+      if (b - a < 50) return false;
+      const int x = keyAt(i), y = keyAt(i - 1);
+      int p = i - 1;
+      if (i - a >= 2) {
+        uint64_t m0, m1;
+        masks([=](int q, int k) { return q < i - 1 && !(x < k); }, m0, m1);
+        p = m1 ? 64 + highbit(m1) + 1 : m0 ? highbit(m0) + 1 : 0;
+      }
+      int r = i;
+      if (i + 1 < b) {
+        uint64_t m0, m1;
+        masks([=](int q, int k) { return q > i && q < b && !(k < y); }, m0, m1);
+        r = m0 ? lowbit(m0) - 1 : m1 ? 64 + lowbit(m1) - 1 : b - 1;
+      }
+      move(i, p);
+      move(i, r);
+      tlo = p < tlo ? p : tlo;
+      thi = r > thi ? r : thi;
+    }
+    return false;
+  }
+  KS_HD int choose(int a, int b, int& hint) const {
+    const int l = b - a, i = a + l / 4, j = a + l / 4 * 2, k = a + l / 4 * 3;
+    int s0 = 0, s1 = 0, s2 = 0, s3 = 0, s4 = 0, s5 = 0, s6 = 0, s7 = 0, s8 = 0;
+    if (l >= 8) {
+      s1 = keyAt(i);
+      s4 = keyAt(j);
+      s7 = keyAt(k);
+      if (l >= 50) {
+        s0 = keyAt(i - 1); s2 = keyAt(i + 1);
+        s3 = keyAt(j - 1); s5 = keyAt(j + 1);
+        s6 = keyAt(k - 1); s8 = keyAt(k + 1);
+      }
+    }
+    return choose_pivot_medians(a, b, hint, s0, s1, s2, s3, s4, s5, s6, s7, s8);
+  }
+  KS_HD int count(int a, int b, int pk, bool below_or_eq) const {
+    uint64_t m0, m1;
+    masks([=](int p, int k) { return p >= a && p < b && (below_or_eq ? k <= pk : k < pk); }, m0, m1);
+    return popc(m0) + popc(m1);
+  }
+  KS_HD int hoare(int l0, int m, int r1, int pk, bool eq) {
+    uint64_t L0, L1, R0, R1;
+    masks([=](int p, int k) { return p >= l0 && p < m && (eq ? k > pk : k >= pk); }, L0, L1);
+    masks([=](int p, int k) { return p >= m && p < r1 && (eq ? k <= pk : k < pk); }, R0, R1);
+    const int nL = popc(L0) + popc(L1);
+    if (nL != popc(R0) + popc(R1)) {
+      bail = 1;
+      return 0;
+    }
+    for (int t = 0; t < nL; t++) {
+      int i, j;
+      if (L0) { i = lowbit(L0); L0 &= L0 - 1; }
+      else { i = 64 + lowbit(L1); L1 &= L1 - 1; }
+      if (R1) { const int h = highbit(R1); j = 64 + h; R1 &= ~(1ull << h); }
+      else { const int h = highbit(R0); j = h; R0 &= ~(1ull << h); }
+      swap(i, j);
+    }
+    return nL;
+  }
+  KS_HD int partition(int a, int b, int pivot, bool& already) {
+    swap(a, pivot);
+    const int pk = keyAt(a);
+    const int j = a + count(a + 1, b, pk, false);
+    already = hoare(a + 1, j + 1, b, pk, false) == 0;
+    swap(j, a);
+    return j;
+  }
+  KS_HD int partition_equal(int a, int b, int pivot) {
+    swap(a, pivot);
+    const int pk = keyAt(a);
+    const int m = a + 1 + count(a + 1, b, pk, true);
+    hoare(a + 1, m, b, pk, true);
+    return m;
+  }
+  KS_HD void leaf_half(Vec& kh, Vec& vh, int a, int b) {
+    Vec rank;
+    W::each([&](int l) { W::at(rank, l) = 0; });
+    for (int j = a; j < b; j++) {
+      const int kj = W::rdl(kh, j);
+      W::each([&](int l) {
+        const int mk = W::get(kh, l);
+        W::at(rank, l) += kj < mk || (kj == mk && j < l) ? 1 : 0;
+      });
+    }
+    const auto dst = [&](int l) { return l >= a && l < b ? a + W::get(rank, l) : l; };
+    kh = W::scatter(kh, dst);
+    vh = W::scatter(vh, dst);
+  }
+  KS_HD void leaf(int a, int b) {
+    if (b - a < 2) return;
+    if (!TWO || b <= 64) return leaf_half(k0, v0, a, b);
+    if (a >= 64) return leaf_half(k1, v1, a - 64, b - 64);
+    const SortRegsT old = *this;
+    for (int pj = a; pj < b; pj++) {
+      const int kj = old.keyAt(pj), vj = old.valAt(pj);
+      uint64_t m0, m1;
+      old.masks([=](int p, int k) { return p >= a && p < b && (k < kj || (k == kj && p < pj)); }, m0, m1);
+      const int d = a + popc(m0) + popc(m1);
+      setKey(d, kj);
+      setVal(d, vj);
+    }
+  }
+  struct Proxy {
+    SortRegsT* s;
+    bool val;
+    struct Ref {
+      SortRegsT* s;
+      bool val;
+      int p;
+      KS_HD operator int32_t() const { return val ? s->valAt(p) : s->keyAt(p); }
+      KS_HD Ref& operator=(int32_t x) {
+        if (val) s->setVal(p, x);
+        else s->setKey(p, x);
+        return *this;
+      }
+      KS_HD Ref& operator=(const Ref& o) { return *this = (int32_t)o; }
+    };
+    KS_HD Ref operator[](int p) const { return Ref{s, val, p}; }
+  };
+
+  KS_HD void heap(int a, int b) {
+    GoSortT<Proxy> g{Proxy{this, false}, Proxy{this, true}};
+    g.heapSort(a, b);
+    heaps++;
+  }
+
+  KS_HD void pdq(int resumePivot) {
+    Vec fa, fb, fl, ff;
+    const int maxsp = 2 * GoSortT<int32_t*>::bitsLen((uint32_t)n) + 2;
+    int budget = 4 * n + 8;
+    const int lim0 = GoSortT<int32_t*>::bitsLen((uint32_t)n);
+    W::each([&](int l) {
+      W::at(fa, l) = 0;
+      W::at(fb, l) = n;
+      W::at(fl, l) = lim0;
+      W::at(ff, l) = 3;
+    });
+    int sp = 1;
+    bool resume = resumePivot >= 0;
+    int dummy_lo = 0, dummy_hi = 0;
+    while (sp > 0) {
+      sp--;
+      int a = W::rdl(fa, sp), b = W::rdl(fb, sp), limit = W::rdl(fl, sp);
+      const int flags = W::rdl(ff, sp);
+      bool wasBalanced = flags & 1, wasPartitioned = (flags >> 1) & 1;
+      for (;;) {
+        if (--budget < 0) {
+          bail = 1;
+          return;
+        }
+        const int length = b - a;
+        int pivot;
+        if (resume) {
+          resume = false;
+          pivot = resumePivot;
+        } else {
+          if (length <= 12) {
+            leaf(a, b);
+            break;
+          }
+          if (limit == 0) {
+            heap(a, b);
+            break;
+          }
+          if (!wasBalanced) {
+            GoSortT<Proxy> g{Proxy{this, false}, Proxy{this, true}};
+            g.breakPatterns(a, b);
+            breaks++;
+            limit--;
+          }
+          int hint = 0;
+          pivot = choose(a, b, hint);
+          if (hint == 2) {
+            reverse(a, b);
+            pivot = (b - 1) - (pivot - a);
+            hint = 1;
+          }
+          if (wasBalanced && wasPartitioned && hint == 1 && pis(a, b, dummy_lo, dummy_hi)) break;
+        }
+        if (a > 0 && !(keyAt(a - 1) < keyAt(pivot))) {
+          a = partition_equal(a, b, pivot);
+          if (bail) return;
+          continue;
+        }
+        bool already = false;
+        const int mid = partition(a, b, pivot, already);
+        if (bail) return;
+        wasPartitioned = already;
+        const int leftLen = mid - a, rightLen = b - mid, thr = length / 8;
+        if (sp + 2 > maxsp) {
+          bail = 1;
+          return;
+        }
+        int c0a, c0b, c1a, c1b;
+        if (leftLen < rightLen) {
+          wasBalanced = leftLen >= thr;
+          c0a = mid + 1; c0b = b; c1a = a; c1b = mid;
+        } else {
+          wasBalanced = rightLen >= thr;
+          c0a = a; c0b = mid; c1a = mid + 1; c1b = b;
+        }
+        const int f0 = (int)wasBalanced | ((int)wasPartitioned << 1);
+        W::each([&, c0a, c0b, c1a, c1b, limit, f0, sp](int l) {
+          const bool m0 = l == sp, m1 = l == sp + 1;
+          W::at(fa, l) = m0 ? c0a : m1 ? c1a : W::get(fa, l);
+          W::at(fb, l) = m0 ? c0b : m1 ? c1b : W::get(fb, l);
+          W::at(fl, l) = m0 || m1 ? limit : W::get(fl, l);
+          W::at(ff, l) = m0 ? f0 : m1 ? 3 : W::get(ff, l);
+        });
+        sp += 2;
+        break;
+      }
+    }
+  }
+  KS_HD uint32_t general(int pivot) {
+    int tlo = n, thi = -1;
+    bool done = false;
+    if (pivot >= 0) done = pis(0, n, tlo, thi);
+    if (!done) {
+      pdq(pivot);
+      tlo = 0;
+      thi = n - 1;
+    }
+    if (bail) return 0;
+    return (uint32_t)tlo | (uint32_t)(thi + 1) << 15 | (uint32_t)done << 30 | 1u << 31;
+  }
+};
+constexpr uint32_t kSortRegsDone = 1u << 31;
+
+struct SortRegsHostOps {
+  struct Vec { int32_t x[64]; };
+  template <class F> static void each(F f) { for (int l = 0; l < 64; l++) f(l); }
+  static int32_t& at(Vec& v, int l) { return v.x[l]; }
+  static int32_t get(const Vec& v, int l) { return v.x[l]; }
+  static int32_t rdl(const Vec& v, int l) { return v.x[l & 63]; }
+  template <class F> static uint64_t ballot(F p) {
+    uint64_t m = 0;
+    for (int l = 0; l < 64; l++) m |= p(l) ? 1ull << l : 0ull;
+    return m;
+  }
+  template <class F> static Vec gather(const Vec& v, F src) {
+    Vec r;
+    for (int l = 0; l < 64; l++) r.x[l] = v.x[src(l) & 63];
+    return r;
+  }
+  template <class F> static Vec scatter(const Vec& v, F dst) {
+    Vec r;
+    for (int l = 0; l < 64; l++) r.x[l] = INT32_MIN;
+    for (int l = 0; l < 64; l++) r.x[dst(l) & 63] = v.x[l];
+    return r;
+  }
+};
+
+inline int sort_regs_model(int n, int32_t* keys, int32_t* order, bool two, int* path) {
+  int pivot = -1;
+  if (n > 12) {
+    GoSort g{keys, order};
+    int hint = 0;
+    const int pv = g.choosePivot(0, n, hint);
+    if (hint == 1) pivot = pv;
+  }
+  uint32_t word = 0;
+  int breaks = 0, heaps = 0;
+  const bool fits = n <= (two ? kSortRegsMax : 64);
+  if (fits) {
+    const auto run = [&](auto& rs) {
+      rs.load(n, [&](int p) { return keys[p]; }, [&](int p) { return order[p]; });
+      word = rs.general(pivot);
+      breaks = rs.breaks;
+      heaps = rs.heaps;
+      if (word) rs.store([&](int p, int k, int v) { keys[p] = k; order[p] = v; });
+    };
+    if (two) {
+      SortRegsT<SortRegsHostOps, true> rs;
+      run(rs);
+    } else {
+      SortRegsT<SortRegsHostOps, false> rs;
+      run(rs);
+    }
+  }
+  if (path) *path = (word ? 1 : fits ? 2 : 3) | breaks << 8 | heaps << 20;
+  if (word) return word >> 30 & 1 ? 0 : 1;
+  GoSortExact g{GoSort{keys, order}};
+  g.run(n);
+  return 1;
+}
+
+}
diff --git a/karpenter-sigs_amd/karpenter_amd/scheduler.py b/karpenter-sigs_amd/karpenter_amd/scheduler.py
--- a/karpenter-sigs_amd/karpenter_amd/scheduler.py
+++ b/karpenter-sigs_amd/karpenter_amd/scheduler.py
@@ -160,7 +160,7 @@
     return out
 
 
-def claim_sort_probe(keys, order, claim_tpl, claim_head, mode=0, pos=-1, device=0):
+def claim_sort_probe(keys, order, claim_tpl, claim_head, mode=0, pos=-1, device=0, path=False):
     import numpy as np
 
     k = np.array(keys, dtype=np.int32)
@@ -173,6 +173,14 @@
     pt = np.zeros(n, dtype=np.int32)
     ph = np.zeros((n, r), dtype=np.int64)
     how = ctypes.c_int(-1)
+    if path or device < -1:
+        pth = ctypes.c_int(0)
+        lib().ks_claim_sort_probe_path.argtypes = ([ctypes.c_int] * 5 + [ctypes.c_void_p] * 6 +
+                                                   [ctypes.POINTER(ctypes.c_int)] * 2)
+        _check(lib().ks_claim_sort_probe_path(device, mode, pos, n, r, k.ctypes.data, o.ctypes.data, ct.ctypes.data,
+                                              ch.ctypes.data, pt.ctypes.data, ph.ctypes.data, ctypes.byref(how),
+                                              ctypes.byref(pth)))
+        return (k, o, pt, ph, how.value, pth.value) if path else (k, o, pt, ph, how.value)
     lib().ks_claim_sort_probe.argtypes = [ctypes.c_int] * 5 + [ctypes.c_void_p] * 6 + [ctypes.POINTER(ctypes.c_int)]
     _check(lib().ks_claim_sort_probe(device, mode, pos, n, r, k.ctypes.data, o.ctypes.data, ct.ctypes.data,
                                      ch.ctypes.data, pt.ctypes.data, ph.ctypes.data, ctypes.byref(how)))
```

New measurement: 8.073 million pods/s (median of 6 runs). +4.4%, better.
